# rsjahnige/CRYSTALS-Kyber

Hardware: AMD Instinct MI355X
Metric: ML-KEM-768 encaps+decaps/sec at batch 2^20; achieved HBM GB/s vs peak (higher is better)
Workload: dtype u32+f32 (64-bit Keccak lanes as 2 x u32; mod-3329 arithmetic exact on integers < 2^24 in the fp32 pipe; u8/u16 I/O)

## Files before the change

### crystals-kyber_amd/csrc/mlkem_keyset.hpp

```cpp
#pragma once
#include "mlkem_pipeline.hpp"

namespace mlkem {

constexpr int32_t KS_ERR_ARG = -101;

struct KeysetView {
    const uint8_t* keys = nullptr;
    size_t key_stride = 0;
    size_t ek_off = 0;
    const uint8_t* h = nullptr;
    const uint16_t* At = nullptr;
    size_t n_keys = 0;
    bool has_dk = false;
};

struct KeysetLimits {
    size_t enc_max_k[3] = {1536, 1024, 768}, dec_max_k[3] = {3072, 2048, 3072};
    size_t enc_lat_k[3] = {256, 512, 256}, dec_lat_k[3] = {384, 256, 256};
    size_t enc_max(int k) const { return enc_max_k[k - 2]; }
    size_t dec_max(int k) const { return dec_max_k[k - 2]; }
    size_t enc_lat(int k) const { return enc_lat_k[k - 2]; }
    size_t dec_lat(int k) const { return dec_lat_k[k - 2]; }
    void set_all(size_t max_items, size_t lat_items) {
        for (int i = 0; i < 3; i++) {
            if (max_items != (size_t)-1) enc_max_k[i] = dec_max_k[i] = max_items;
            if (lat_items != (size_t)-1) enc_lat_k[i] = dec_lat_k[i] = lat_items;
        }
    }
};

__device__ __forceinline__ size_t keyset_key(const uint32_t* __restrict__ idx, size_t n_keys, size_t item) {
    if (!idx) return 0;
    const size_t k = idx[item];
    return k < n_keys ? k : 0;
}

__global__ void __launch_bounds__(WAVE, MLKEM_KECCAK_MINWAVES) k_hash_g_keyset(size_t n, const uint32_t* __restrict__ idx, size_t n_keys,
                                                                               const uint8_t* __restrict__ m, const uint8_t* __restrict__ hs,
                                                                               uint8_t* __restrict__ Kout, uint8_t* __restrict__ r_ws) {
    const size_t item = (size_t)blockIdx.x * WAVE + lane_id();
    const size_t it = item < n ? item : n - 1;
    uint32_t mm[8], hh[8], w[8];
    load32(m, 32, it, mm);
    load32(hs, 32, keyset_key(idx, n_keys, it), hh);
    KeccakState s;
    lane_G64(s, mm, hh);
    if (item < n) {
        MLKEM_STATE_WORDS8(s, 0, w)
        store32(Kout, 32, item, w);
        MLKEM_STATE_WORDS8(s, 8, w)
        store32(r_ws, 32, item, w);
    }
}

__global__ void __launch_bounds__(256) k_keyset_gather32(size_t n, const uint32_t* __restrict__ idx, size_t n_keys, const uint8_t* __restrict__ src,
                                                         size_t stride, uint32_t* __restrict__ dst) {
    const size_t g = (size_t)blockIdx.x * blockDim.x + threadIdx.x;
    if (g >= 8 * n) return;
    const size_t item = g >> 3;
    dst[g] = reinterpret_cast<const uint32_t*>(src + keyset_key(idx, n_keys, item) * stride)[g & 7];
}

template <int K, int CLEN, int JRATE>
__global__ void __launch_bounds__(WAVE, MLKEM_KECCAK_MINWAVES) k_hash_decaps_keyset(size_t n, const uint32_t* __restrict__ idx, size_t n_keys,
                                                                                    const uint8_t* __restrict__ hs, uint8_t* __restrict__ z_ws,
                                                                                    const uint8_t* __restrict__ c, const uint8_t* __restrict__ m_ws,
                                                                                    uint8_t* __restrict__ Kp_ws, uint8_t* __restrict__ r_ws,
                                                                                    uint8_t* __restrict__ Kbar_ws) {
    __shared__ __attribute__((aligned(16))) uint2 stage[STAGE_QWORDS];
    const size_t item0 = (size_t)blockIdx.x * WAVE;
    KeccakState s;
    uint32_t h[8], w[8];
    {
        MsgView mv{z_ws, 32, 32, c, CLEN, CLEN};
        wave_sponge_absorb<JRATE, 0x1F>(s, stage, mv, item0, n);
        const size_t i2 = item0 + (size_t)lane_id_fresh();
        if (i2 < n) {
            MLKEM_STATE_WORDS8(s, 0, w)
            store32(Kbar_ws, 32, i2, w);
            uint32_t* zr = reinterpret_cast<uint32_t*>(z_ws + i2 * 32);
#pragma unroll
            for (int q = 0; q < 8; q++) zr[q] = 0u;
        }
    }
    uint32_t mm[8];
    const size_t i3 = item0 + (size_t)lane_id_fresh(), it = i3 < n ? i3 : n - 1;
    load32(m_ws, 32, it, mm);
    load32(hs, 32, keyset_key(idx, n_keys, it), h);
    lane_G64(s, mm, h);
    const size_t item = item0 + (size_t)lane_id_fresh();
    if (item < n) {
        MLKEM_STATE_WORDS8(s, 0, w)
        store32(Kp_ws, 32, item, w);
        MLKEM_STATE_WORDS8(s, 8, w)
        store32(r_ws, 32, item, w);
    }
}

template <int K, int ETA1, int DU, int DV, bool COMPARE>
__global__ void __launch_bounds__(WAVE * KPKE2_WAVES, kpke2_minwaves(K))
k_encrypt2_keyset(size_t n, const uint32_t* __restrict__ idx, size_t n_keys, const uint8_t* __restrict__ ek, size_t ek_stride,
                  const uint16_t* __restrict__ At, const uint8_t* __restrict__ msg, const uint8_t* __restrict__ prf, uint8_t* __restrict__ c_out,
                  const uint8_t* __restrict__ c_in, const uint8_t* __restrict__ Kp, const uint8_t* __restrict__ Kbar, uint8_t* __restrict__ Kout) {
    __shared__ K2Lds<K + 1> lds_all[KPKE2_WAVES];
    const int wv = wave_id();
    const size_t item0 = 2 * ((size_t)blockIdx.x * KPKE2_WAVES + wv);
    if (item0 >= n) return;
    const size_t h = (size_t)(lane_id() >> 5), item = item0 + h < n ? item0 + h : item0;
    const size_t key = keyset_key(idx, n_keys, item);
    encrypt2_body<K, ETA1, DU, DV, COMPARE>(lds_all[wv].xch, item0, n, ek + key * ek_stride, 0, msg, At + key * (size_t)(K * K * 256), prf,
                                            c_out, c_in, Kp, Kbar, Kout, (int32_t*)nullptr, 0);
}

template <int K, int DU, int DV>
__global__ void __launch_bounds__(64 * KPKE4_WAVES, kpke4_minwaves(K)) k_decrypt4_keyset(size_t n, const uint32_t* __restrict__ idx, size_t n_keys,
                                                                                       const uint8_t* __restrict__ dk, size_t dk_stride,
                                                                                       const uint8_t* __restrict__ c, uint8_t* __restrict__ m_out) {
    const size_t quad = (size_t)blockIdx.x * KPKE4_WAVES + wave_id();
    if (4 * quad >= n) return;
    const size_t item_raw = 4 * quad + (size_t)rntt_lane().p, item = item_raw < n ? item_raw : n - 1;
    decrypt4_body<K, DU, DV>(quad, n, dk + keyset_key(idx, n_keys, item) * dk_stride, 0, c, m_out);
}

__global__ void __launch_bounds__(256) k_keyset_fix(size_t n, const uint32_t* __restrict__ idx, size_t n_keys, uint8_t* __restrict__ c,
                                                    unsigned c_len, uint8_t* __restrict__ Kout, int32_t* __restrict__ status) {
    for (size_t i = (size_t)blockIdx.x * blockDim.x + threadIdx.x; i < n; i += (size_t)gridDim.x * blockDim.x) {
        const bool bad = idx && (size_t)idx[i] >= n_keys;
        if (status) status[i] = bad ? KS_ERR_ARG : 0;
        if (!bad) continue;
        uint32_t* k = reinterpret_cast<uint32_t*>(Kout + i * 32);
        for (int w = 0; w < 8; w++) k[w] = 0;
        if (c) {
            uint32_t* cw = reinterpret_cast<uint32_t*>(c + i * c_len);
            for (unsigned w = 0; w < c_len / 4; w++) cw[w] = 0;
        }
    }
}

__global__ void __launch_bounds__(256) k_keyset_status_or(size_t n, const int32_t* __restrict__ status, uint32_t* __restrict__ out) {
    uint32_t v = 0;
    for (size_t i = (size_t)blockIdx.x * blockDim.x + threadIdx.x; i < n; i += (size_t)gridDim.x * blockDim.x) v |= (uint32_t)status[i];
    if (v) atomicOr(out, v);
}

template <int K, int ETA1>
struct __attribute__((aligned(16))) KeysetHand {
    uint8_t prf[(2 * K + 1) * (ETA1 == 3 ? 192 : 128)];
    uint8_t r[32], m[32], Kp[32], Kbar[32];
};

__device__ __forceinline__ void keyset_small_reject(size_t item, uint8_t* c, unsigned c_len, uint8_t* Kout, int32_t* status) {
    const unsigned l = (unsigned)lane_id();
    if (l < 8) reinterpret_cast<uint32_t*>(Kout + item * 32)[l] = 0;
    if (c)
        for (unsigned w = l; w < c_len / 4; w += WAVE) reinterpret_cast<uint32_t*>(c + item * c_len)[w] = 0;
    if (l == 0 && status) status[item] = KS_ERR_ARG;
}

template <int K, int ETA1, int DU, int DV, int NW>
__global__ void __launch_bounds__(WAVE * NW)
k_encaps_keyset_small(size_t n, const uint32_t* __restrict__ idx, size_t n_keys, const uint8_t* __restrict__ ek, size_t ek_stride,
                      const uint8_t* __restrict__ hs, const uint16_t* __restrict__ At, const uint8_t* __restrict__ m, uint8_t* __restrict__ c,
                      uint8_t* __restrict__ Kout, int32_t* __restrict__ status, int prf_rate) {
    __shared__ K2Lds<K + 1> xl;
    __shared__ KeysetHand<K, ETA1> hand;
    __shared__ uint2 rc_tables[NW][WK_RC_ENTRIES];
    __shared__ SmallSync sy;
    constexpr unsigned CLEN = 32 * (DU * K + DV);
    const int wv = wave_id();
    const size_t item = blockIdx.x;
    if (item >= n) return;
    const size_t key = idx ? (size_t)idx[item] : 0;
    if (key >= n_keys) {
        if (wv == 0) keyset_small_reject(item, c, CLEN, Kout, status);
        return;
    }
    const uint8_t* my_ek = ek + key * ek_stride;
    WkLane cst;
    wk_lane_init(cst, rc_tables[wave_id()]);
    if (threadIdx.x == 0) { sy.next_job = K * K; sy.jobs_done = 0; sy.r_ready = 0; sy.kbar_ready = 0; }
    block_barrier();
    if (wv == 0) {
        const int i = wk_index();
        uint2 v;
        v.x = 0; v.y = 0;
        if (i >= 0 && i < 4) v = reinterpret_cast<const uint2*>(m + item * 32)[i];
        else if (i >= 4 && i < 8) v = reinterpret_cast<const uint2*>(hs + key * 32)[i - 4];
        WkState a;
        a.lo = v.x; a.hi = v.y;
        if (i == 8) { a.lo = 0x06u; a.hi = 0x80000000u; }
        wk_permute(a, cst);
        uint2 o;
        o.x = a.lo; o.y = a.hi;
        if (wk_primary() && i < 4) reinterpret_cast<uint2*>(Kout + item * 32)[i] = o;
        else if (wk_primary() && i < 8) reinterpret_cast<uint2*>(hand.r)[i - 4] = o;
        flag_signal(&sy.r_ready);
    }
    small_jobs<K, ETA1>(sy, cst, nullptr, true, nullptr, hand.r, hand.prf, 2 * K + 1, (unsigned)prf_rate, nullptr);
    if (wv != 0) return;
    flag_wait(&sy.jobs_done, (uint32_t)(2 * K + 1));
    encrypt1_body<K, ETA1, DU, DV, false>(xl.xch, my_ek, m + item * 32, At + key * (size_t)(K * K * 256), hand.prf, c + item * CLEN, nullptr,
                                          nullptr, nullptr, nullptr, nullptr);
    if (lane_id() == 0 && status) status[item] = 0;
    wave_lds_fence();
    wave_zero_lds(hand);
    wave_zero_lds(xl);
#ifdef MLKEM_EMU_LDS_PROBE
    if (lane_id() == 0) { MLKEM_EMU_LDS_PROBE(&hand, sizeof hand); MLKEM_EMU_LDS_PROBE(&xl, sizeof xl); }
#endif
}

template <int K, int ETA1, int DU, int DV, int JRATE, int NW>
__global__ void __launch_bounds__(WAVE * NW)
k_decaps_keyset_small(size_t n, const uint32_t* __restrict__ idx, size_t n_keys, const uint8_t* __restrict__ dk, size_t dk_stride,
                      const uint8_t* __restrict__ hs, const uint16_t* __restrict__ At, const uint8_t* __restrict__ c, uint8_t* __restrict__ Kout,
                      int32_t* __restrict__ status, int prf_rate) {
    static_assert(NW >= 2, "roles of waves 0 and 1");
    __shared__ K2Lds<K + 1> xl;
    __shared__ KeysetHand<K, ETA1> hand;
    __shared__ uint2 rc_tables[NW][WK_RC_ENTRIES];
    __shared__ SmallSync sy;
    constexpr unsigned DK = 768 * K + 96, CLEN = 32 * (DU * K + DV);
    const int wv = wave_id();
    const size_t item = blockIdx.x;
    if (item >= n) return;
    const size_t key = idx ? (size_t)idx[item] : 0;
    if (key >= n_keys) {
        if (wv == 0) keyset_small_reject(item, nullptr, CLEN, Kout, status);
        return;
    }
    const uint8_t* my_dk = dk + key * dk_stride;
    const uint8_t* my_c = c + item * CLEN;
    WkLane cst;
    wk_lane_init(cst, rc_tables[wave_id()]);
    const int i = wk_index();
    const bool prim = wk_primary();
    if (threadIdx.x == 0) { sy.next_job = K * K; sy.jobs_done = 0; sy.r_ready = 0; sy.kbar_ready = 0; }
    block_barrier();
    if (wv == 0) {
        decrypt4_body<K, DU, DV>(0, 1, my_dk, (size_t)DK, my_c, hand.m);
        wave_global_fence();
        uint2 v;
        v.x = 0; v.y = 0;
        if (i >= 0 && i < 4) v = reinterpret_cast<const uint2*>(hand.m)[i];
        else if (i >= 4 && i < 8) v = reinterpret_cast<const uint2*>(hs + key * 32)[i - 4];
        WkState a;
        a.lo = v.x; a.hi = v.y;
        if (i == 8) { a.lo = 0x06u; a.hi = 0x80000000u; }
        wk_permute(a, cst);
        uint2 o;
        o.x = a.lo; o.y = a.hi;
        if (prim && i < 4) reinterpret_cast<uint2*>(hand.Kp)[i] = o;
        else if (prim && i < 8) reinterpret_cast<uint2*>(hand.r)[i - 4] = o;
        flag_signal(&sy.r_ready);
    } else if (wv == 1) {
        WkState a;
        wk_absorb<JRATE, 0x1F>(a, cst, my_dk + 768 * K + 64, 32, my_c, 32 + CLEN);
        uint2 o;
        o.x = a.lo; o.y = a.hi;
        if (prim && i < 4) reinterpret_cast<uint2*>(hand.Kbar)[i] = o;
        flag_signal(&sy.kbar_ready);
    }
    small_jobs<K, ETA1>(sy, cst, nullptr, true, nullptr, hand.r, hand.prf, 2 * K + 1, (unsigned)prf_rate, nullptr);
    if (wv != 0) return;
    flag_wait(&sy.jobs_done, (uint32_t)(2 * K + 1));
    encrypt1_body<K, ETA1, DU, DV, true>(xl.xch, my_dk + 384 * K, hand.m, At + key * (size_t)(K * K * 256), hand.prf, nullptr, my_c, hand.Kp,
                                         hand.Kbar, Kout + item * 32, nullptr, &sy.kbar_ready);
    if (lane_id() == 0 && status) status[item] = 0;
    wave_lds_fence();
    wave_zero_lds(hand);
    wave_zero_lds(xl);
#ifdef MLKEM_EMU_LDS_PROBE
    if (lane_id() == 0) { MLKEM_EMU_LDS_PROBE(&hand, sizeof hand); MLKEM_EMU_LDS_PROBE(&xl, sizeof xl); }
#endif
}

inline size_t keyset_table_bytes_per_key(const ParamSet& p, bool has_dk) {
    return (has_dk ? (size_t)p.dk_len : (size_t)p.ek_len) + 32 + (size_t)(p.k * p.k) * 512;
}

template <int K>
inline void keyset_import_run(stream_t st, const ParamSet& p, const KeysetView& ks, uint8_t* hs, uint16_t* At, int32_t* status,
                              uint32_t* status_or, const Workspace& ws) {
    const size_t n = ks.n_keys;
    zero_u32x2(st, status_or);
    if (status) {
        const uint8_t* ek = ks.has_dk ? nullptr : ks.keys;
        const uint8_t* dk = ks.has_dk ? ks.keys : nullptr;
        check_keys_dispatch(st, p.set, n, ek, dk, nullptr, nullptr, status, nullptr, min_sz(n, ws.cap), ws);
        launch("k_keyset_status_or", k_keyset_status_or, min_sz(ceil_div(n, 256), 1024), 256u, st, n, (const int32_t*)status, status_or);
    }
    hash_launch(st, 0, n, ks.keys + ks.ek_off, p.ek_len, ks.key_stride, hs);
    for (size_t c0 = 0; c0 < n; c0 += ws.cap) {
        const size_t cn = min_sz(ws.cap, n - c0);
        Workspace w = ws;
        w.A = At + c0 * (size_t)(K * K * 256);
        launch_sample_split(st, p, cn, 0, ks.keys + c0 * ks.key_stride + ks.ek_off + 384 * K, ks.key_stride, 1, nullptr, 0, 0, w);
    }
}

inline void keyset_seed_run(stream_t st, const ParamSet& p, size_t n, const uint8_t* seed, uint8_t* dk, uint8_t* tmp, const Workspace& ws) {
    uint8_t *d = tmp, *z = d + n * 32, *ek = z + n * 32;
    launch("k_seed_split", k_seed_split, ceil_div(4 * n, 256), 256, st, n, reinterpret_cast<const uint4*>(seed), reinterpret_cast<uint4*>(d),
           reinterpret_cast<uint4*>(z));
    keygen_dispatch(st, p.set, n, d, z, ek, dk, ws);
}

template <int K, int ETA1, int DU, int DV>
inline void encaps_keyset_run(stream_t st, const ParamSet& p, const KeysetView& ks, size_t n, const uint32_t* idx, const uint8_t* m, uint8_t* c,
                              uint8_t* Kout, int32_t* status, const Workspace& ws, const KeysetLimits& lim) {
    if (n == 0) return;
    const uint8_t* ek = ks.keys + ks.ek_off;
    if (n <= lim.enc_max(K)) {
        const int rate = ws.fips ? 136 : 168;
        if (n <= lim.enc_lat(K))
            launch("k_encaps_keyset_small", k_encaps_keyset_small<K, ETA1, DU, DV, SMALL_WAVES>, n, WAVE * SMALL_WAVES, st, n, idx, ks.n_keys, ek,
                   ks.key_stride, ks.h, ks.At, m, c, Kout, status, rate);
        else
            launch("k_encaps_keyset_small", k_encaps_keyset_small<K, ETA1, DU, DV, SMALL_WAVES_DENSE>, n, WAVE * SMALL_WAVES_DENSE, st, n, idx,
                   ks.n_keys, ek, ks.key_stride, ks.h, ks.At, m, c, Kout, status, rate);
        return;
    }
    for (size_t h0 = 0; h0 < n; h0 += ws.hcap) {
        const size_t hn = min_sz(ws.hcap, n - h0);
        const uint32_t* idh = idx ? idx + h0 : nullptr;
        launch("k_hash_g_keyset", k_hash_g_keyset, ceil_div(hn, WAVE), WAVE, st, hn, idh, ks.n_keys, m + h0 * 32, ks.h, Kout + h0 * 32, ws.r);
        for (size_t c0 = 0; c0 < hn; c0 += ws.cap) {
            const size_t cn = min_sz(ws.cap, hn - c0), i0 = h0 + c0;
            launch_sample_split(st, p, 0, cn, nullptr, 0, 1, ws.r + c0 * 32, 2 * K + 1, K, ws);
            launch("k_encrypt_keyset", k_encrypt2_keyset<K, ETA1, DU, DV, false>, ceil_div(ceil_div(cn, 2), KPKE2_WAVES), WAVE * KPKE2_WAVES, st, cn,
                   idx ? idx + i0 : nullptr, ks.n_keys, ek, ks.key_stride, ks.At, m + i0 * 32, (const uint8_t*)ws.prf, c + i0 * p.c_len,
                   (const uint8_t*)nullptr, (const uint8_t*)nullptr, (const uint8_t*)nullptr, (uint8_t*)nullptr);
        }
    }
    if (idx || status)
        launch("k_keyset_fix", k_keyset_fix, min_sz(ceil_div(n, 256), 1024), 256u, st, n, idx, ks.n_keys, c, p.c_len, Kout, status);
}

template <int K, int ETA1, int DU, int DV>
inline void decaps_keyset_run(stream_t st, const ParamSet& p, const KeysetView& ks, size_t n, const uint32_t* idx, const uint8_t* c,
                              uint8_t* Kout, int32_t* status, const Workspace& ws, const KeysetLimits& lim) {
    constexpr int CLEN = 32 * (DU * K + DV);
    if (n == 0) return;
    if (n <= lim.dec_max(K)) {
        const int rate = ws.fips ? 136 : 168;
#define MLKEM_DKS(JR, NW) launch("k_decaps_keyset_small", k_decaps_keyset_small<K, ETA1, DU, DV, JR, NW>, n, WAVE * NW, st, n, idx, ks.n_keys, \
                                 ks.keys, ks.key_stride, ks.h, ks.At, c, Kout, status, rate)
        if (!ws.fips && n <= lim.dec_lat(K)) MLKEM_DKS(168, SMALL_WAVES);
        else if (!ws.fips) MLKEM_DKS(168, SMALL_WAVES_DENSE);
        else if (n <= lim.dec_lat(K)) MLKEM_DKS(136, SMALL_WAVES);
        else MLKEM_DKS(136, SMALL_WAVES_DENSE);
#undef MLKEM_DKS
        return;
    }
    for (size_t h0 = 0; h0 < n; h0 += ws.hcap) {
        const size_t hn = min_sz(ws.hcap, n - h0);
        const uint32_t* idh = idx ? idx + h0 : nullptr;
        const uint8_t* ch = c + h0 * p.c_len;
        launch("k_decrypt_keyset", k_decrypt4_keyset<K, DU, DV>, ceil_div(ceil_div(hn, 4), KPKE4_WAVES), 64 * KPKE4_WAVES, st, hn, idh, ks.n_keys,
               ks.keys, ks.key_stride, ch, ws.m);
        launch("k_keyset_gather32", k_keyset_gather32, ceil_div(8 * hn, 256), 256u, st, hn, idh, ks.n_keys, ks.keys + 768 * K + 64, ks.key_stride,
               reinterpret_cast<uint32_t*>(ws.rho));
        if (!ws.fips)
            launch("k_hash_decaps_keyset", k_hash_decaps_keyset<K, CLEN, 168>, ceil_div(hn, WAVE), WAVE, st, hn, idh, ks.n_keys, ks.h,
                   ws.rho, ch, (const uint8_t*)ws.m, ws.Kp, ws.r, ws.Kbar);
        else
            launch("k_hash_decaps_keyset", k_hash_decaps_keyset<K, CLEN, 136>, ceil_div(hn, WAVE), WAVE, st, hn, idh, ks.n_keys, ks.h,
                   ws.rho, ch, (const uint8_t*)ws.m, ws.Kp, ws.r, ws.Kbar);
        for (size_t c0 = 0; c0 < hn; c0 += ws.cap) {
            const size_t cn = min_sz(ws.cap, hn - c0), i0 = h0 + c0;
            launch_sample_split(st, p, 0, cn, nullptr, 0, 1, ws.r + c0 * 32, 2 * K + 1, K, ws);
            launch("k_encrypt_cmp_keyset", k_encrypt2_keyset<K, ETA1, DU, DV, true>, ceil_div(ceil_div(cn, 2), KPKE2_WAVES), WAVE * KPKE2_WAVES, st,
                   cn, idx ? idx + i0 : nullptr, ks.n_keys, ks.keys + 384 * K, ks.key_stride, ks.At, (const uint8_t*)(ws.m + c0 * 32),
                   (const uint8_t*)ws.prf, (uint8_t*)nullptr, c + i0 * p.c_len, (const uint8_t*)(ws.Kp + c0 * 32), (const uint8_t*)(ws.Kbar + c0 * 32),
                   Kout + i0 * 32);
        }
    }
    if (idx || status)
        launch("k_keyset_fix", k_keyset_fix, min_sz(ceil_div(n, 256), 1024), 256u, st, n, idx, ks.n_keys, (uint8_t*)nullptr, p.c_len, Kout, status);
}

inline int keyset_import_dispatch(stream_t st, const ParamSet& p, const KeysetView& ks, uint8_t* hs, uint16_t* At, int32_t* status,
                                  uint32_t* status_or, const Workspace& ws) {
    switch (p.set) {
    case 512: keyset_import_run<2>(st, p, ks, hs, At, status, status_or, ws); break;
    case 768: keyset_import_run<3>(st, p, ks, hs, At, status, status_or, ws); break;
    default: keyset_import_run<4>(st, p, ks, hs, At, status, status_or, ws); break;
    }
    return 0;
}
inline int encaps_keyset_dispatch(stream_t st, const ParamSet& p, const KeysetView& ks, size_t n, const uint32_t* idx, const uint8_t* m,
                                  uint8_t* c, uint8_t* K, int32_t* status, const Workspace& ws, const KeysetLimits& lim) {
    switch (p.set) {
    case 512: encaps_keyset_run<2, 3, 10, 4>(st, p, ks, n, idx, m, c, K, status, ws, lim); break;
    case 768: encaps_keyset_run<3, 2, 10, 4>(st, p, ks, n, idx, m, c, K, status, ws, lim); break;
    default: encaps_keyset_run<4, 2, 11, 5>(st, p, ks, n, idx, m, c, K, status, ws, lim); break;
    }
    return 0;
}
inline int decaps_keyset_dispatch(stream_t st, const ParamSet& p, const KeysetView& ks, size_t n, const uint32_t* idx, const uint8_t* c,
                                  uint8_t* K, int32_t* status, const Workspace& ws, const KeysetLimits& lim) {
    switch (p.set) {
    case 512: decaps_keyset_run<2, 3, 10, 4>(st, p, ks, n, idx, c, K, status, ws, lim); break;
    case 768: decaps_keyset_run<3, 2, 10, 4>(st, p, ks, n, idx, c, K, status, ws, lim); break;
    default: decaps_keyset_run<4, 2, 11, 5>(st, p, ks, n, idx, c, K, status, ws, lim); break;
    }
    return 0;
}

}
```

### crystals-kyber_amd/csrc/mlkem_kpke2.hpp

```cpp
#pragma once
#include "mlkem_arith.hpp"
#include "mlkem_rntt.hpp"
#include <type_traits>

namespace mlkem {

#ifndef MLKEM_KPKE2_WAVES
#define MLKEM_KPKE2_WAVES 1
#endif
constexpr int KPKE2_WAVES = MLKEM_KPKE2_WAVES;
#ifdef MLKEM_KPKE2_MINWAVES
constexpr int kpke2_minwaves(int) { return MLKEM_KPKE2_MINWAVES; }
#else
constexpr int kpke2_minwaves(int k) { return k == 2 ? 4 : k == 3 ? 3 : 2; }
#endif

template <int NP>
struct __attribute__((aligned(16))) K2Lds {
    float2 xch[NP][2][128];
};

__device__ __forceinline__ int k2_slot(int pair) { return pair ^ ((pair & 64) ? 0x15 : 0) ^ ((pair & 32) ? 0x0A : 0); }
enum K2Layout { K2_LA = 0, K2_LB = 1, K2_LC = 2, K2_NAT = 3 };
__device__ __forceinline__ int k2_blk(int t) { return (((t >> 2) & 3) << 3) | ((t >> 4) << 2) | (t & 3); }
__device__ __forceinline__ int k2_lc_hi(int t) { return (((t >> 2) & 3) << 2) | ((t >> 4) << 1) | ((t >> 1) & 1); }
template <int LAYOUT>
__device__ __forceinline__ int k2_pair(int t, int j) {
    if constexpr (LAYOUT == K2_LA) return (j << 5) | t;
    else if constexpr (LAYOUT == K2_LB) return ((t >> 3) << 5) | (j << 3) | (t & 7);
    else if constexpr (LAYOUT == K2_LC) return (k2_lc_hi(t) << 3) | (j << 1) | (t & 1);
    else return (k2_blk(t) << 2) | j;
}
template <int LAYOUT>
__device__ __forceinline__ void k2_write(float2* xh, int t, const v2f (&p)[4]) {
#pragma unroll
    for (int j = 0; j < 4; j++) {
        float2 v;
        v.x = p[j].x; v.y = p[j].y;
        xh[k2_slot(k2_pair<LAYOUT>(t, j))] = v;
    }
}
template <int LAYOUT>
__device__ __forceinline__ void k2_read(const float2* xh, int t, v2f (&p)[4]) {
#pragma unroll
    for (int j = 0; j < 4; j++) {
        const float2 v = xh[k2_slot(k2_pair<LAYOUT>(t, j))];
        p[j] = v2f{v.x, v.y};
    }
}
template <int FROM, int TO, int NP>
__device__ __forceinline__ void k2_exchange(float2 (*xch)[2][128], int h, int t, v2f (&p)[NP][4]) {
#pragma unroll
    for (int q = 0; q < NP; q++) k2_write<FROM>(xch[q][h], t, p[q]);
    wave_lds_fence();
#pragma unroll
    for (int q = 0; q < NP; q++) k2_read<TO>(xch[q][h], t, p[q]);
    wave_lds_fence();
}

struct K2Tw {
    Tw b0, b1, b2, c0, c1, c2, d0, d1;
};
__device__ __forceinline__ void k2_twiddles_fwd(K2Tw& w, int t) {
    const Tw* z = ZETA_F.z;
    const int b = t >> 3, c = k2_lc_hi(t), n = k2_blk(t);
    w.b0 = z[4 + b]; w.b1 = z[8 + 2 * b]; w.b2 = z[9 + 2 * b];
    w.c0 = z[16 + c]; w.c1 = z[32 + 2 * c]; w.c2 = z[33 + 2 * c];
    w.d0 = z[64 + 2 * n]; w.d1 = z[65 + 2 * n];
}
__device__ __forceinline__ void k2_twiddles_inv(K2Tw& w, int t) {
    const Tw* z = ZETA_F.z;
    const int b = t >> 3, c = k2_lc_hi(t), n = k2_blk(t);
    w.d0 = z[127 - 2 * n]; w.d1 = z[126 - 2 * n];
    w.c1 = z[63 - 2 * c]; w.c2 = z[62 - 2 * c]; w.c0 = z[31 - c];
    w.b1 = z[15 - 2 * b]; w.b2 = z[14 - 2 * b]; w.b0 = z[7 - b];
}

template <int N>
__device__ __forceinline__ void k2_shoup_n(const Tw (&z)[N], v2f (&b)[N]) {
    v2f km[N], nk[N];
#pragma unroll
    for (int i = 0; i < N; i++) km[i] = fma2(b[i], splat2(z[i].zq), splat2(F_MAGIC));
#pragma unroll
    for (int i = 0; i < N; i++) nk[i] = fma2(km[i], splat2(-F_Q), splat2(F_MAGIC_Q));
#pragma unroll
    for (int i = 0; i < N; i++) b[i] = fma2(b[i], splat2(z[i].z), nk[i]);
}
template <int N>
__device__ __forceinline__ void k2_fred_n(v2f (&x)[N]) {
    v2f k[N];
#pragma unroll
    for (int i = 0; i < N; i++) k[i] = fma2(x[i], splat2(F_INVQ), splat2(F_MAGIC));
#pragma unroll
    for (int i = 0; i < N; i++) k[i] = k[i] - splat2(F_MAGIC);
#pragma unroll
    for (int i = 0; i < N; i++) x[i] = fma2(k[i], splat2(-F_Q), x[i]);
}
template <int N, bool GS>
__device__ __forceinline__ void k2_bfly_n(v2f (&a)[N], v2f (&b)[N], const Tw (&z)[N]) {
    if constexpr (!GS) {
        k2_shoup_n<N>(z, b);
#pragma unroll
        for (int i = 0; i < N; i++) { const v2f tt = b[i]; b[i] = a[i] - tt; a[i] = a[i] + tt; }
    } else {
        v2f d[N];
#pragma unroll
        for (int i = 0; i < N; i++) d[i] = b[i] - a[i];
#pragma unroll
        for (int i = 0; i < N; i++) a[i] = a[i] + b[i];
        k2_shoup_n<N>(z, d);
#pragma unroll
        for (int i = 0; i < N; i++) b[i] = d[i];
    }
}
template <int NP, bool GS>
__device__ __forceinline__ void k2_layer_hi(v2f (&p)[NP][4], Tw z) {
    v2f a[2 * NP], b[2 * NP];
    Tw zz[2 * NP];
#pragma unroll
    for (int q = 0; q < NP; q++) { a[2 * q] = p[q][0]; b[2 * q] = p[q][2]; a[2 * q + 1] = p[q][1]; b[2 * q + 1] = p[q][3]; zz[2 * q] = z; zz[2 * q + 1] = z; }
    k2_bfly_n<2 * NP, GS>(a, b, zz);
#pragma unroll
    for (int q = 0; q < NP; q++) { p[q][0] = a[2 * q]; p[q][2] = b[2 * q]; p[q][1] = a[2 * q + 1]; p[q][3] = b[2 * q + 1]; }
}
template <int NP, bool GS>
__device__ __forceinline__ void k2_layer_lo(v2f (&p)[NP][4], Tw z01, Tw z23) {
    v2f a[2 * NP], b[2 * NP];
    Tw zz[2 * NP];
#pragma unroll
    for (int q = 0; q < NP; q++) { a[2 * q] = p[q][0]; b[2 * q] = p[q][1]; a[2 * q + 1] = p[q][2]; b[2 * q + 1] = p[q][3]; zz[2 * q] = z01; zz[2 * q + 1] = z23; }
    k2_bfly_n<2 * NP, GS>(a, b, zz);
#pragma unroll
    for (int q = 0; q < NP; q++) { p[q][0] = a[2 * q]; p[q][1] = b[2 * q]; p[q][2] = a[2 * q + 1]; p[q][3] = b[2 * q + 1]; }
}
template <int NP, int R0, int R1>
__device__ __forceinline__ void k2_fred_pairs(v2f (&p)[NP][4]) {
    v2f x[2 * NP];
#pragma unroll
    for (int q = 0; q < NP; q++) { x[2 * q] = p[q][R0]; x[2 * q + 1] = p[q][R1]; }
    k2_fred_n<2 * NP>(x);
#pragma unroll
    for (int q = 0; q < NP; q++) { p[q][R0] = x[2 * q]; p[q][R1] = x[2 * q + 1]; }
}

template <int NP>
__device__ __forceinline__ void k2_ntt(v2f (&p)[NP][4], float2 (*xch)[2][128], int h, int t, const K2Tw& w) {
    k2_layer_hi<NP, false>(p, FZ1);
    k2_layer_lo<NP, false>(p, FZ2, FZ3);
    k2_exchange<K2_LA, K2_LB, NP>(xch, h, t, p);
    k2_layer_hi<NP, false>(p, w.b0);
    k2_layer_lo<NP, false>(p, w.b1, w.b2);
    k2_exchange<K2_LB, K2_LC, NP>(xch, h, t, p);
    k2_layer_hi<NP, false>(p, w.c0);
    k2_layer_lo<NP, false>(p, w.c1, w.c2);
    k2_exchange<K2_LC, K2_NAT, NP>(xch, h, t, p);
    k2_layer_lo<NP, false>(p, w.d0, w.d1);
}
template <int NP>
__device__ __forceinline__ void k2_intt(v2f (&p)[NP][4], float2 (*xch)[2][128], int h, int t, const K2Tw& w) {
    k2_layer_lo<NP, true>(p, w.d0, w.d1);
    k2_fred_pairs<NP, 0, 2>(p);
    k2_exchange<K2_NAT, K2_LC, NP>(xch, h, t, p);
    k2_layer_lo<NP, true>(p, w.c1, w.c2);
    k2_layer_hi<NP, true>(p, w.c0);
    k2_fred_pairs<NP, 0, 1>(p);
    k2_exchange<K2_LC, K2_LB, NP>(xch, h, t, p);
    k2_layer_lo<NP, true>(p, w.b1, w.b2);
    k2_layer_hi<NP, true>(p, w.b0);
    k2_fred_pairs<NP, 0, 1>(p);
    k2_exchange<K2_LB, K2_LA, NP>(xch, h, t, p);
    k2_layer_lo<NP, true>(p, FZ3, FZ2);
    {
        v2f sm[2 * NP], df[2 * NP];
        Tw zs[2 * NP], zd[2 * NP];
#pragma unroll
        for (int q = 0; q < NP; q++)
#pragma unroll
            for (int m = 0; m < 2; m++) {
                sm[2 * q + m] = p[q][m] + p[q][m + 2];
                df[2 * q + m] = p[q][m + 2] - p[q][m];
                zs[2 * q + m] = F_INV128; zd[2 * q + m] = F_INV128_Z1;
            }
        k2_shoup_n<2 * NP>(zs, sm);
        k2_shoup_n<2 * NP>(zd, df);
#pragma unroll
        for (int q = 0; q < NP; q++)
#pragma unroll
            for (int m = 0; m < 2; m++) { p[q][m] = sm[2 * q + m]; p[q][m + 2] = df[2 * q + m]; }
    }
    k2_exchange<K2_LA, K2_NAT, NP>(xch, h, t, p);
}

template <int ETA>
struct K2CbdRaw {
    uint32_t w[ETA == 2 ? 1 : 2];
};
template <int ETA>
__device__ __forceinline__ void k2_cbd_load_la(const uint8_t* prf, int t, K2CbdRaw<ETA>& r) {
    if constexpr (ETA == 2) {
        r.w[0] = (uint32_t)prf[t] | ((uint32_t)prf[t + 32] << 8) | ((uint32_t)prf[t + 64] << 16) | ((uint32_t)prf[t + 96] << 24);
    } else {
        uint32_t f[4];
#pragma unroll
        for (int j = 0; j < 4; j++) {
            const int o = ((3 * t) >> 1) + 48 * j;
            f[j] = (((uint32_t)prf[o] | ((uint32_t)prf[o + 1] << 8)) >> (4 * (t & 1))) & 0xFFFu;
        }
        r.w[0] = f[0] | (f[1] << 12);
        r.w[1] = f[2] | (f[3] << 12);
    }
}
__device__ __forceinline__ uint32_t k2_cbd_load_nat2(const uint8_t* prf, int t) { return reinterpret_cast<const uint32_t*>(prf)[t]; }
template <bool BIASED = false>
__device__ __forceinline__ void k2_cbd2_eval8(uint32_t t, v2f (&p)[4]) {
    const uint32_t s = (t & 0x55555555u) + ((t >> 1) & 0x55555555u);
    const uint32_t d = ((s & 0x33333333u) + 0x22222222u) - ((s >> 2) & 0x33333333u);
    const uint32_t lo = d & 0x0F0F0F0Fu, hi = (d >> 4) & 0x0F0F0F0Fu;
    float fl[4] = {(float)(lo & 0xFFu), (float)((lo >> 8) & 0xFFu), (float)((lo >> 16) & 0xFFu), (float)(lo >> 24)};
    float fh[4] = {(float)(hi & 0xFFu), (float)((hi >> 8) & 0xFFu), (float)((hi >> 16) & 0xFFu), (float)(hi >> 24)};
#ifndef MLKEM_EMU
    asm volatile("" : "+v"(fl[0]), "+v"(fl[1]), "+v"(fl[2]), "+v"(fl[3]), "+v"(fh[0]), "+v"(fh[1]), "+v"(fh[2]), "+v"(fh[3]));
#endif
#pragma unroll
    for (int j = 0; j < 4; j++) {
        if constexpr (BIASED) p[j] = v2f{fl[j], fh[j]};
        else p[j] = v2f{fl[j], fh[j]} - splat2(2.0f);
    }
}
template <int ETA>
__device__ __forceinline__ void k2_cbd_eval(const K2CbdRaw<ETA>& r, v2f (&p)[4]) {
    if constexpr (ETA == 2) {
        k2_cbd2_eval8<false>(r.w[0], p);
    } else {
        float a[4], b[4];
        cbd_eval_f<3>(r.w[0], a);
        cbd_eval_f<3>(r.w[1], b);
        p[0] = v2f{a[0], a[1]}; p[1] = v2f{a[2], a[3]}; p[2] = v2f{b[0], b[1]}; p[3] = v2f{b[2], b[3]};
    }
}

__device__ __forceinline__ void k2_gamma(const v2f (&y)[4], Tw d0, Tw d1, float (&yg)[4]) {
    yg[0] = fmulmod_shoup(d0, y[0].y);
    yg[1] = fmulmod_shoup(tw_neg(d0), y[1].y);
    yg[2] = fmulmod_shoup(d1, y[2].y);
    yg[3] = fmulmod_shoup(tw_neg(d1), y[3].y);
}
__device__ __forceinline__ void k2_basemul_acc(v2f (&acc)[4], const v2f (&a)[4], const v2f (&y)[4], const float (&yg)[4]) {
    v2f c[4];
#pragma unroll
    for (int j = 0; j < 4; j++) c[j] = fma2(splat2(a[j].x), y[j], acc[j]);
#pragma unroll
    for (int j = 0; j < 4; j++) {
        c[j].x = __builtin_fmaf(a[j].y, yg[j], c[j].x);
        c[j].y = __builtin_fmaf(a[j].y, y[j].x, c[j].y);
    }
    k2_fred_n<4>(c);
#pragma unroll
    for (int j = 0; j < 4; j++) acc[j] = c[j];
}

__device__ __forceinline__ void k2_unpack16(const uint4 v, v2f (&p)[4]) {
    const uint32_t w[4] = {v.x, v.y, v.z, v.w};
#pragma unroll
    for (int j = 0; j < 4; j++) p[j] = v2f{(float)(w[j] & 0xFFFFu), (float)(w[j] >> 16)};
}
__device__ __forceinline__ void k2_decode12(uint32_t w0, uint32_t w1, uint32_t w2, v2f (&p)[4]) {
    const uint32_t c0 = w0 & 0xFFFu, c1 = (w0 >> 12) & 0xFFFu, c2 = __builtin_amdgcn_alignbit(w1, w0, 24) & 0xFFFu, c3 = (w1 >> 4) & 0xFFFu;
    const uint32_t c4 = (w1 >> 16) & 0xFFFu, c5 = __builtin_amdgcn_alignbit(w2, w1, 28) & 0xFFFu, c6 = (w2 >> 8) & 0xFFFu, c7 = w2 >> 20;
    p[0] = v2f{(float)c0, (float)c1}; p[1] = v2f{(float)c2, (float)c3}; p[2] = v2f{(float)c4, (float)c5}; p[3] = v2f{(float)c6, (float)c7};
}

__device__ __forceinline__ uint32_t f_bits(float x) {
    union { float f; uint32_t u; } v;
    v.f = x;
    return v.u;
}
template <int D, bool BIASED = false>
__device__ __forceinline__ void k2_compress4(const v2f (&x)[4], unsigned (&c)[8]) {
    v2f tt[4], k0m[4], k0[4], r[4], km[4];
#pragma unroll
    for (int j = 0; j < 4; j++) tt[j] = fma2(x[j], splat2((float)(1 << D)), splat2(BIASED ? -(float)(2 << D) : 0.0f));
#pragma unroll
    for (int j = 0; j < 4; j++) k0m[j] = fma2(tt[j], splat2(F_INVQ), splat2(F_MAGIC));
#pragma unroll
    for (int j = 0; j < 4; j++) k0[j] = k0m[j] - splat2(F_MAGIC);
#pragma unroll
    for (int j = 0; j < 4; j++) r[j] = fma2(k0[j], splat2(-F_Q), tt[j]);
#pragma unroll
    for (int j = 0; j < 4; j++) km[j] = fma2(r[j], splat2(F_INVQ), splat2(F_MAGIC));
#pragma unroll
    for (int j = 0; j < 4; j++) {
        c[2 * j] = (f_bits(k0m[j].x) + f_bits(km[j].x)) & ((1u << D) - 1u);
        c[2 * j + 1] = (f_bits(k0m[j].y) + f_bits(km[j].y)) & ((1u << D) - 1u);
    }
}

__device__ __forceinline__ uint32_t k2_swap1(uint32_t v) {
#ifdef MLKEM_EMU
    return (uint32_t)emu_quad_shfl((int)v, (int)((threadIdx.x & 3) ^ 1));
#else
    return (uint32_t)__builtin_amdgcn_mov_dpp((int)v, 0xB1, 0xF, 0xF, true);
#endif
}
__device__ __forceinline__ uint32_t k2_prev_in_quad(uint32_t v) {
#ifdef MLKEM_EMU
    const int l = (int)(threadIdx.x & 3);
    return (uint32_t)emu_quad_shfl((int)v, l ? l - 1 : l);
#else
    return (uint32_t)__builtin_amdgcn_mov_dpp((int)v, 0x90, 0xF, 0xF, true);
#endif
}
__device__ __forceinline__ uint32_t k2_shl_hi(uint32_t hi, uint32_t lo, unsigned s) {
    return s ? __builtin_amdgcn_alignbit(hi, lo, 32u - s) : hi;
}

template <int D>
struct K2Piece {
    static_assert(D == 4 || D == 5 || D == 10 || D == 11 || D == 12, "ciphertext / key encodings of ML-KEM");
    static constexpr int NW = D == 4 ? 1 : D == 5 ? 2 : 3;
    uint32_t w[NW];
    static __device__ __forceinline__ int first(int t) {
        if constexpr (D == 4) return t;
        else if constexpr (D == 12) return 3 * t;
        else if constexpr (D == 10) return 5 * (t >> 1) + ((t & 1) ? 3 : 0);
        else if constexpr (D == 11) return 11 * (t >> 2) + ((88 * (t & 3)) >> 5);
        else return 5 * (t >> 2) + (t & 3);
    }
    static __device__ __forceinline__ int count(int t) {
        if constexpr (D == 4) return 1;
        else if constexpr (D == 12) return 3;
        else if constexpr (D == 10) return (t & 1) ? 2 : 3;
        else if constexpr (D == 11) return (t & 3) ? 3 : 2;
        else return (t & 3) == 3 ? 2 : 1;
    }
};
template <int D>
__device__ __forceinline__ void k2_encode(const unsigned (&c)[8], int t, K2Piece<D>& o) {
    if constexpr (D == 4) {
        o.w[0] = c[0] | (c[1] << 4) | (c[2] << 8) | (c[3] << 12) | (c[4] << 16) | (c[5] << 20) | (c[6] << 24) | (c[7] << 28);
    } else if constexpr (D == 12) {
        o.w[0] = c[0] | (c[1] << 12) | (c[2] << 24);
        o.w[1] = (c[2] >> 8) | (c[3] << 4) | (c[4] << 16) | (c[5] << 28);
        o.w[2] = (c[5] >> 4) | (c[6] << 8) | (c[7] << 20);
    } else if constexpr (D == 10) {
        const uint32_t v0 = c[0] | (c[1] << 10) | (c[2] << 20) | (c[3] << 30);
        const uint32_t v1 = (c[3] >> 2) | (c[4] << 8) | (c[5] << 18) | (c[6] << 28);
        const uint32_t v2 = (c[6] >> 4) | (c[7] << 6);
        const uint32_t other0 = k2_swap1(v0);
        const unsigned sh = (t & 1) ? 16u : 0u;
        o.w[0] = __builtin_amdgcn_alignbit(v1, v0, sh);
        o.w[1] = __builtin_amdgcn_alignbit(v2, v1, sh);
        o.w[2] = v2 | (other0 << 16);
    } else if constexpr (D == 11) {
        const uint32_t v0 = c[0] | (c[1] << 11) | (c[2] << 22);
        const uint32_t v1 = (c[2] >> 10) | (c[3] << 1) | (c[4] << 12) | (c[5] << 23);
        const uint32_t v2 = (c[5] >> 9) | (c[6] << 2) | (c[7] << 13);
        const int j = t & 3;
        const unsigned sh = (88u * (unsigned)j) & 31u;
        const uint32_t e0 = v0 << sh, e1 = k2_shl_hi(v1, v0, sh), e2 = k2_shl_hi(v2, v1, sh), e3 = k2_shl_hi(0u, v2, sh);
        const uint32_t tail = j == 0 ? e2 : e3;
        const uint32_t prev = k2_prev_in_quad(tail);
        o.w[0] = e0 | (j ? prev : 0u);
        o.w[1] = e1;
        o.w[2] = e2;
    } else {
        const uint32_t v0 = c[0] | (c[1] << 5) | (c[2] << 10) | (c[3] << 15) | (c[4] << 20) | (c[5] << 25) | (c[6] << 30);
        const uint32_t v1 = (c[6] >> 2) | (c[7] << 3);
        const int j = t & 3;
        const unsigned sh = 8u * (unsigned)j;
        const uint32_t e0 = v0 << sh, e1 = k2_shl_hi(v1, v0, sh);
        const uint32_t prev = k2_prev_in_quad(e1);
        o.w[0] = e0 | (j ? prev : 0u);
        o.w[1] = e1;
    }
}
template <int D>
__device__ __forceinline__ void k2_piece_load(const uint8_t* poly, int t, K2Piece<D>& o) {
    const uint32_t* g = reinterpret_cast<const uint32_t*>(poly) + K2Piece<D>::first(t);
#pragma unroll
    for (int i = 0; i < K2Piece<D>::NW; i++) o.w[i] = i < K2Piece<D>::count(t) ? stream_load4(g + i) : 0u;
}
template <int D>
__device__ __forceinline__ void k2_piece_store(uint8_t* poly, int t, const K2Piece<D>& o) {
    uint32_t* g = reinterpret_cast<uint32_t*>(poly) + K2Piece<D>::first(t);
#pragma unroll
    for (int i = 0; i < K2Piece<D>::NW; i++)
        if (i < K2Piece<D>::count(t)) g[i] = o.w[i];
}
template <int D>
__device__ __forceinline__ uint32_t k2_piece_diff(int t, const K2Piece<D>& a, const K2Piece<D>& ref) {
    uint32_t d = 0;
#pragma unroll
    for (int i = 0; i < K2Piece<D>::NW; i++)
        if (i < K2Piece<D>::count(t)) d |= a.w[i] ^ ref.w[i];
    return d;
}
template <int D, bool COMPARE, bool BIASED = false>
__device__ __forceinline__ uint32_t k2_emit(const v2f (&p)[4], int t, uint8_t* out, const K2Piece<D>& ref, bool store) {
    unsigned c[8];
    k2_compress4<D, BIASED>(p, c);
    K2Piece<D> o;
    k2_encode<D>(c, t, o);
    if constexpr (COMPARE) return k2_piece_diff<D>(t, o, ref);
    if (store) k2_piece_store<D>(out, t, o);
    return 0;
}

template <int K, int ETA1, int DU, int DV, bool COMPARE>
__device__ __forceinline__ void
encrypt2_body(float2 (*xch)[2][128], size_t item0, size_t n, const uint8_t* __restrict__ ek, size_t ek_stride, const uint8_t* __restrict__ msg,
              const uint16_t* __restrict__ A, const uint8_t* __restrict__ prf, uint8_t* __restrict__ c_out, const uint8_t* __restrict__ c_in,
              const uint8_t* __restrict__ Kp, const uint8_t* __restrict__ Kbar, uint8_t* __restrict__ Kout, int32_t* __restrict__ mod_status,
              size_t a_stride) {
    const int l = lane_id(), h = l >> 5, t = l & 31, nb = k2_blk(t);
    const bool valid = item0 + (size_t)h < n;
    const unsigned hh = valid ? (unsigned)h : 0u;
    constexpr unsigned PS = (ETA1 == 3) ? 192 : 128, CLEN = 32 * (DU * K + DV), PRFLEN = (2 * K + 1) * PS;
    const uint8_t* my_prf = prf + item0 * (size_t)PRFLEN + (size_t)(hh * PRFLEN);
    const uint8_t* my_ek = ek + item0 * ek_stride + (size_t)(hh * (unsigned)ek_stride);
    const uint16_t* my_A = A + item0 * a_stride + (size_t)(hh * (unsigned)a_stride);
    uint8_t* my_c = COMPARE ? nullptr : c_out + item0 * CLEN + (size_t)(hh * CLEN);
    const uint8_t* my_cin = COMPARE ? c_in + item0 * CLEN + (size_t)(hh * CLEN) : nullptr;
    const size_t item = item0 + hh;

    K2CbdRaw<ETA1> raw_y[K];
#pragma unroll
    for (int b = 0; b < K; b++) k2_cbd_load_la<ETA1>(my_prf + b * PS, t, raw_y[b]);
    uint4 a_all[K + 1][K];
#pragma unroll
    for (int a = 0; a < K; a++)
#pragma unroll
        for (int b = 0; b < K; b++) a_all[a][b] = *reinterpret_cast<const uint4*>(my_A + (a * K + b) * 256 + 8 * nb);
#pragma unroll
    for (int b = 0; b < K; b++) {
        const uint32_t* gp = reinterpret_cast<const uint32_t*>(my_ek + 384 * b) + 3 * nb;
        a_all[K][b].x = stream_load4(gp); a_all[K][b].y = stream_load4(gp + 1); a_all[K][b].z = stream_load4(gp + 2); a_all[K][b].w = 0u;
    }
    uint32_t raw_e[K + 1];
#pragma unroll
    for (int a = 0; a <= K; a++) raw_e[a] = k2_cbd_load_nat2(my_prf + (K + a) * PS, nb);
    const unsigned mb = msg[item * 32 + nb];

    v2f yh[K][4];
    float yg[K][4];
    {
        K2Tw tw;
        k2_twiddles_fwd(tw, t);
#pragma unroll
        for (int b = 0; b < K; b++) k2_cbd_eval<ETA1>(raw_y[b], yh[b]);
        k2_ntt<K>(yh, xch, h, t, tw);
#pragma unroll
        for (int b = 0; b < K; b++) {
            k2_fred_n<4>(yh[b]);
            k2_gamma(yh[b], tw.d0, tw.d1, yg[b]);
        }
    }
    uint32_t diff = 0;
    bool over = false;
    constexpr int NG = K + 1;
    v2f acc[NG][4];
    K2Piece<DU> cu_ref[NG];
    K2Piece<DV> cv_ref;
#pragma unroll
    for (int a = 0; a < NG; a++) {
#pragma unroll
        for (int j = 0; j < 4; j++) acc[a][j] = splat2(0.f);
#pragma unroll
        for (int b = 0; b < K; b++) {
            v2f av[4];
            if (a < K) {
                k2_unpack16(a_all[a][b], av);
            } else {
                k2_decode12(a_all[a][b].x, a_all[a][b].y, a_all[a][b].z, av);
#pragma unroll
                for (int j = 0; j < 4; j++) over = over || (av[j].x >= F_Q) || (av[j].y >= F_Q);
            }
            k2_basemul_acc(acc[a], av, yh[b], yg[b]);
        }
    }
    if constexpr (COMPARE) {
#pragma unroll
        for (int a = 0; a < NG; a++) {
            if (a < K) k2_piece_load<DU>(my_cin + a * 32 * DU, nb, cu_ref[a]);
            else k2_piece_load<DV>(my_cin + K * 32 * DU, nb, cv_ref);
        }
    }
    {
        K2Tw twi;
        k2_twiddles_inv(twi, t);
        k2_intt<NG>(acc, xch, h, t, twi);
    }
#pragma unroll
    for (int a = 0; a < NG; a++) {
        v2f e[4];
        k2_cbd2_eval8<true>(raw_e[a], e);
#pragma unroll
        for (int j = 0; j < 4; j++) acc[a][j] = acc[a][j] + e[j];
        if (a < K) {
            diff |= k2_emit<DU, COMPARE, true>(acc[a], nb, COMPARE ? nullptr : my_c + a * 32 * DU, cu_ref[a], valid);
        } else {
#pragma unroll
            for (int j = 0; j < 4; j++)
                acc[a][j] = acc[a][j] + v2f{((mb >> (2 * j)) & 1u) ? 1665.0f : 0.0f, ((mb >> (2 * j + 1)) & 1u) ? 1665.0f : 0.0f};
            diff |= k2_emit<DV, COMPARE, true>(acc[a], nb, COMPARE ? nullptr : my_c + K * 32 * DU, cv_ref, valid);
        }
    }
    if (mod_status) {
        const unsigned long long bal = __ballot(over);
        const bool bad = ((bal >> (32 * h)) & 0xFFFFFFFFull) != 0;
        if (t == 0 && valid) mod_status[item] = bad ? -4 : 0;
    }
    if constexpr (COMPARE) {
        const unsigned long long bal = __ballot(diff != 0);
        const uint32_t reject = ((bal >> (32 * h)) & 0xFFFFFFFFull) != 0 ? 0xFFFFFFFFu : 0u;
        if (t < 8 && valid) {
            const uint32_t kp = reinterpret_cast<const uint32_t*>(Kp + item * 32)[t];
            const uint32_t kb = reinterpret_cast<const uint32_t*>(Kbar + item * 32)[t];
            reinterpret_cast<uint32_t*>(Kout + item * 32)[t] = (kp & ~reject) | (kb & reject);
        }
    }
}
template <int K, int ETA1, int DU, int DV, bool COMPARE, bool A_T = false>
__device__ __forceinline__ void
encrypt1_body(float2 (*xch)[2][128], const uint8_t* __restrict__ ek, const uint8_t* __restrict__ msg, const uint16_t* __restrict__ A,
              const uint8_t* __restrict__ prf, uint8_t* __restrict__ c_out, const uint8_t* __restrict__ c_in, const uint8_t* __restrict__ Kp,
              const uint8_t* Kbar, uint8_t* __restrict__ Kout, int32_t* __restrict__ mod_status,
              const uint32_t* kbar_flag = nullptr) {
    const int l = lane_id(), h = l >> 5, t = l & 31, nb = k2_blk(t);
    constexpr unsigned PS = (ETA1 == 3) ? 192 : 128;
    constexpr int NG = K + 1, NL = (NG + 1) / 2;
    auto kind = [](int i) constexpr { return 2 * i + 1 < K ? 0 : (2 * i < K ? 1 : 2); };

    K2CbdRaw<ETA1> raw_y[K];
#pragma unroll
    for (int b = 0; b < K; b++) k2_cbd_load_la<ETA1>(prf + b * PS, t, raw_y[b]);
    uint4 a_all[NL][K];
    uint32_t raw_e[NL];
#pragma unroll
    for (int i = 0; i < NL; i++) {
        const int a = kind(i) == 2 ? K : 2 * i + h;
        const bool is_v = kind(i) == 2 || (kind(i) == 1 && h == 1);
#pragma unroll
        for (int b = 0; b < K; b++) {
            if (is_v) {
                const uint32_t* gp = reinterpret_cast<const uint32_t*>(ek + 384 * b) + 3 * nb;
                a_all[i][b].x = gp[0]; a_all[i][b].y = gp[1]; a_all[i][b].z = gp[2]; a_all[i][b].w = 0u;
            } else {
                a_all[i][b] = *reinterpret_cast<const uint4*>(A + (A_T ? b * K + a : a * K + b) * 256 + 8 * nb);
            }
        }
        raw_e[i] = k2_cbd_load_nat2(prf + (K + a) * PS, nb);
    }
    const unsigned mb = msg[nb];

    v2f yh[K][4];
    float yg[K][4];
    {
        K2Tw tw;
        k2_twiddles_fwd(tw, t);
#pragma unroll
        for (int b = 0; b < K; b++) k2_cbd_eval<ETA1>(raw_y[b], yh[b]);
        k2_ntt<K>(yh, xch, h, t, tw);
#pragma unroll
        for (int b = 0; b < K; b++) {
            k2_fred_n<4>(yh[b]);
            k2_gamma(yh[b], tw.d0, tw.d1, yg[b]);
        }
    }
    uint32_t diff = 0;
    bool over = false;
    v2f acc[NL][4];
    K2Piece<DU> cu_ref[NL];
    K2Piece<DV> cv_ref;
#pragma unroll
    for (int i = 0; i < NL; i++) {
        const bool is_v = kind(i) == 2 || (kind(i) == 1 && h == 1);
#pragma unroll
        for (int j = 0; j < 4; j++) acc[i][j] = splat2(0.f);
#pragma unroll
        for (int b = 0; b < K; b++) {
            v2f av[4];
            if (is_v) {
                k2_decode12(a_all[i][b].x, a_all[i][b].y, a_all[i][b].z, av);
#pragma unroll
                for (int j = 0; j < 4; j++) over = over || (av[j].x >= F_Q) || (av[j].y >= F_Q);
            } else {
                k2_unpack16(a_all[i][b], av);
            }
            k2_basemul_acc(acc[i], av, yh[b], yg[b]);
        }
    }
    if constexpr (COMPARE) {
#pragma unroll
        for (int i = 0; i < NL; i++) {
            const int a = kind(i) == 2 ? K : 2 * i + h;
            const bool is_v = kind(i) == 2 || (kind(i) == 1 && h == 1);
            if (is_v) k2_piece_load<DV>(c_in + K * 32 * DU, nb, cv_ref);
            else k2_piece_load<DU>(c_in + a * 32 * DU, nb, cu_ref[i]);
        }
    }
    {
        K2Tw twi;
        k2_twiddles_inv(twi, t);
        k2_intt<NL>(acc, xch, h, t, twi);
    }
#pragma unroll
    for (int i = 0; i < NL; i++) {
        const int a = kind(i) == 2 ? K : 2 * i + h;
        const bool is_v = kind(i) == 2 || (kind(i) == 1 && h == 1);
        const bool store = kind(i) != 2 || h == 0;
        v2f e[4];
        k2_cbd2_eval8<true>(raw_e[i], e);
#pragma unroll
        for (int j = 0; j < 4; j++) acc[i][j] = acc[i][j] + e[j];
        if (is_v) {
#pragma unroll
            for (int j = 0; j < 4; j++)
                acc[i][j] = acc[i][j] + v2f{((mb >> (2 * j)) & 1u) ? 1665.0f : 0.0f, ((mb >> (2 * j + 1)) & 1u) ? 1665.0f : 0.0f};
            diff |= k2_emit<DV, COMPARE, true>(acc[i], nb, COMPARE ? nullptr : c_out + K * 32 * DU, cv_ref, store);
        } else {
            diff |= k2_emit<DU, COMPARE, true>(acc[i], nb, COMPARE ? nullptr : c_out + a * 32 * DU, cu_ref[i], store);
        }
    }
    if (mod_status) {
        const bool bad = __ballot(over) != 0;
        if (l == 0) mod_status[0] = bad ? -4 : 0;
    }
    if constexpr (COMPARE) {
        const uint32_t reject = __ballot(diff != 0) != 0 ? 0xFFFFFFFFu : 0u;
        if (kbar_flag) flag_wait(kbar_flag, 1u);
        if (l < 8) {
            const uint32_t kp = reinterpret_cast<const uint32_t*>(Kp)[l];
            const uint32_t kb = reinterpret_cast<const uint32_t*>(Kbar)[l];
            reinterpret_cast<uint32_t*>(Kout)[l] = (kp & ~reject) | (kb & reject);
        }
    }
}

template <int K, int ETA1, int DU, int DV, bool COMPARE>
__global__ void __launch_bounds__(WAVE * KPKE2_WAVES, kpke2_minwaves(K))
k_encrypt2(size_t n, const uint8_t* __restrict__ ek, size_t ek_stride, const uint8_t* __restrict__ msg, const uint16_t* __restrict__ A,
           const uint8_t* __restrict__ prf, uint8_t* __restrict__ c_out, const uint8_t* __restrict__ c_in, const uint8_t* __restrict__ Kp,
           const uint8_t* __restrict__ Kbar, uint8_t* __restrict__ Kout, int32_t* __restrict__ mod_status, size_t a_stride) {
    __shared__ K2Lds<K + 1> lds_all[KPKE2_WAVES];
    const int wv = wave_id();
    const size_t item0 = 2 * ((size_t)blockIdx.x * KPKE2_WAVES + wv);
    if (item0 >= n) return;
    encrypt2_body<K, ETA1, DU, DV, COMPARE>(lds_all[wv].xch, item0, n, ek, ek_stride, msg, A, prf, c_out, c_in, Kp, Kbar, Kout, mod_status, a_stride);
}

__device__ __forceinline__ void k2_canon(const v2f (&p)[4], unsigned (&c)[8]) {
    v2f r[4] = {p[0], p[1], p[2], p[3]};
    k2_fred_n<4>(r);
#pragma unroll
    for (int j = 0; j < 4; j++) {
        const int a = (int)r[j].x, b = (int)r[j].y;
        c[2 * j] = (unsigned)(a + ((a >> 31) & KQ));
        c[2 * j + 1] = (unsigned)(b + ((b >> 31) & KQ));
    }
}

template <int K, int ETA1, bool KEM_DK>
__device__ __forceinline__ void
keygen2_body(float2 (*xch)[2][128], size_t item0, size_t n, const uint16_t* __restrict__ A, const uint8_t* __restrict__ prf,
             const uint8_t* __restrict__ rho, uint8_t* __restrict__ ek, uint8_t* __restrict__ dk) {
    const int l = lane_id(), h = l >> 5, t = l & 31, nb = k2_blk(t);
    const bool valid = item0 + (size_t)h < n;
    const unsigned hh = valid ? (unsigned)h : 0u;
    constexpr unsigned PS = (ETA1 == 3) ? 192 : 128, EK = 384 * K + 32, DK = KEM_DK ? 768 * K + 96 : 384 * K, PRFLEN = 2 * K * PS;
    const uint8_t* my_prf = prf + item0 * (size_t)PRFLEN + (size_t)(hh * PRFLEN);
    const uint16_t* my_A = A + item0 * (size_t)(K * K * 256) + (size_t)(hh * (unsigned)(K * K * 256));
    uint8_t* my_ek = ek + item0 * EK + (size_t)(hh * EK);
    uint8_t* my_dk = dk + item0 * DK + (size_t)(hh * DK);
    const size_t item = item0 + hh;

    K2CbdRaw<ETA1> raw_s[K], raw_e[K];
#pragma unroll
    for (int b = 0; b < K; b++) k2_cbd_load_la<ETA1>(my_prf + b * PS, t, raw_s[b]);
    constexpr bool PF = K >= 3;
    uint4 a_all[K][K];
    if constexpr (PF) {
#pragma unroll
        for (int a = 0; a < K; a++)
#pragma unroll
            for (int b = 0; b < K; b++) a_all[a][b] = *reinterpret_cast<const uint4*>(my_A + (a * K + b) * 256 + 8 * nb);
    }
#pragma unroll
    for (int a = 0; a < K; a++) k2_cbd_load_la<ETA1>(my_prf + (K + a) * PS, t, raw_e[a]);
    const uint32_t rho_w = reinterpret_cast<const uint32_t*>(rho + item * 32)[t & 7];
    K2Tw tw;
    k2_twiddles_fwd(tw, t);
    v2f sh[K][4];
    float sg[K][4];
#pragma unroll
    for (int b = 0; b < K; b++) k2_cbd_eval<ETA1>(raw_s[b], sh[b]);
    k2_ntt<K>(sh, xch, h, t, tw);
#pragma unroll
    for (int b = 0; b < K; b++) {
        k2_fred_n<4>(sh[b]);
        k2_gamma(sh[b], tw.d0, tw.d1, sg[b]);
        unsigned c[8];
        k2_canon(sh[b], c);
        K2Piece<12> o;
        k2_encode<12>(c, nb, o);
        if (valid) k2_piece_store<12>(my_dk + 384 * b, nb, o);
    }
    v2f eh[K][4];
#pragma unroll
    for (int a = 0; a < K; a++) k2_cbd_eval<ETA1>(raw_e[a], eh[a]);
    k2_ntt<K>(eh, xch, h, t, tw);
#pragma unroll
    for (int a = 0; a < K; a++) {
        v2f acc[4] = {splat2(0.f), splat2(0.f), splat2(0.f), splat2(0.f)};
#pragma unroll
        for (int b = 0; b < K; b++) {
            v2f av[4];
            if constexpr (!PF) a_all[a][b] = *reinterpret_cast<const uint4*>(my_A + (a * K + b) * 256 + 8 * nb);
            k2_unpack16(a_all[a][b], av);
            k2_basemul_acc(acc, av, sh[b], sg[b]);
        }
#pragma unroll
        for (int j = 0; j < 4; j++) acc[j] = acc[j] + eh[a][j];
        unsigned c[8];
        k2_canon(acc, c);
        K2Piece<12> o;
        k2_encode<12>(c, nb, o);
        if (valid) {
            k2_piece_store<12>(my_ek + 384 * a, nb, o);
            if constexpr (KEM_DK) k2_piece_store<12>(my_dk + 384 * K + 384 * a, nb, o);
        }
    }
    if (t < 8 && valid) {
        reinterpret_cast<uint32_t*>(my_ek + 384 * K)[t] = rho_w;
        if constexpr (KEM_DK) reinterpret_cast<uint32_t*>(my_dk + 768 * K)[t] = rho_w;
    }
}
template <int K, int ETA1, bool KEM_DK>
__global__ void __launch_bounds__(WAVE * KPKE2_WAVES, K == 2 ? kpke2_minwaves(2) : kpke2_minwaves(K + 1))
k_keygen2(size_t n, const uint16_t* __restrict__ A, const uint8_t* __restrict__ prf, const uint8_t* __restrict__ rho,
          uint8_t* __restrict__ ek, uint8_t* __restrict__ dk) {
    __shared__ K2Lds<K> lds_all[KPKE2_WAVES];
    const int wv = wave_id();
    const size_t item0 = 2 * ((size_t)blockIdx.x * KPKE2_WAVES + wv);
    if (item0 >= n) return;
    keygen2_body<K, ETA1, KEM_DK>(lds_all[wv].xch, item0, n, A, prf, rho, ek, dk);
}

}
```

### crystals-kyber_amd/csrc/mlkem_pipeline.hpp

```cpp
#pragma once
#include "mlkem_kernels.hpp"
#include "mlkem_sampler.hpp"
#include "mlkem_arith.hpp"
#include "mlkem_rntt.hpp"
#include "mlkem_kpke4.hpp"
#include "mlkem_kpke2.hpp"
#include "mlkem_wkeccak.hpp"
#include "mlkem_small.hpp"
#include "mlkem_check.hpp"
#include <stdlib.h>
#ifndef MLKEM_EMU
#include <vector>
#endif

namespace mlkem {

#ifdef MLKEM_EMU
using stream_t = void*;
#else
using stream_t = hipStream_t;
#endif

#ifndef MLKEM_EMU
struct LaunchRecorder {
    struct Rec { const char* label; hipEvent_t a, b; };
    std::vector<Rec> recs;
    bool failed = false;
};
inline LaunchRecorder*& launch_recorder() {
    static thread_local LaunchRecorder* r = nullptr;
    return r;
}
#endif

template <class... KArgs, class... Args>
inline void launch(const char* label, void (*kfn)(KArgs...), size_t grid, unsigned block, stream_t st, Args... args) {
    if (grid == 0) return;
#ifdef MLKEM_EMU
    (void)st; (void)label;
    emu::launch((unsigned)grid, block, [=] { kfn(args...); });
#else
    LaunchRecorder* rec = launch_recorder();
    LaunchRecorder::Rec r{label, nullptr, nullptr};
    bool timed = rec && hipEventCreate(&r.a) == hipSuccess && hipEventCreate(&r.b) == hipSuccess && hipEventRecord(r.a, st) == hipSuccess;
    kfn<<<dim3((unsigned)grid), dim3(block), 0, st>>>(args...);
    if (timed) timed = hipEventRecord(r.b, st) == hipSuccess;
    if (timed) {
        rec->recs.push_back(r);
    } else if (rec) {
        rec->failed = true;
        if (r.a) (void)hipEventDestroy(r.a);
        if (r.b) (void)hipEventDestroy(r.b);
    }
#endif
}

inline void zero_u32x2(stream_t st, uint32_t* p) {
#ifdef MLKEM_EMU
    (void)st;
    p[0] = 0; p[1] = 0;
#else
    (void)hipMemsetAsync(p, 0, 2 * sizeof(uint32_t), st);
#endif
}

struct ParamSet {
    int set, k, eta1, eta2, du, dv;
    unsigned ek_len, dk_len, c_len;
};
inline bool param_set(int set, ParamSet& p) {
    switch (set) {
    case 512: p = {512, 2, 3, 2, 10, 4, 0, 0, 0}; break;
    case 768: p = {768, 3, 2, 2, 10, 4, 0, 0, 0}; break;
    case 1024: p = {1024, 4, 2, 2, 11, 5, 0, 0, 0}; break;
    default: return false;
    }
    p.ek_len = 384u * p.k + 32;
    p.dk_len = 768u * p.k + 96;
    p.c_len = 32u * (p.du * p.k + p.dv);
    return true;
}

struct Workspace {
    uint16_t* A = nullptr;
    uint8_t *prf = nullptr, *r = nullptr, *rho = nullptr, *m = nullptr, *Kp = nullptr, *Kbar = nullptr;
    uint32_t* leftover = nullptr;
    uint32_t* resume = nullptr;
    uint32_t resume_cap = 0;
    size_t cap = 0;
    size_t hcap = 0;
    size_t wide_max = 2048;
    size_t wide_max_k[3] = {4096, 3072, 4096};
    size_t wide_kem(int k) const { return wide_max_k[k - 2]; }
    size_t small_max_k[3] = {1536, 768, 512};
    size_t small_max(int k) const { return small_max_k[k - 2]; }
    size_t small_lat_max = 256;
    size_t small_wide_max = 128;
    unsigned stages = 15;
    int fips = 0;
#ifndef MLKEM_EMU
    hipStream_t side = nullptr;
    hipEvent_t ev_fork = nullptr, ev_join = nullptr;
    bool side_on = true;
#endif
};
struct SideFork {
    stream_t main, side = nullptr;
#ifndef MLKEM_EMU
    hipEvent_t join = nullptr;
#endif
    SideFork(const Workspace& ws, stream_t st, size_t n) : main(st) {
#ifndef MLKEM_EMU
        if (ws.side && ws.side_on && n <= ws.cap && hipEventRecord(ws.ev_fork, st) == hipSuccess && hipStreamWaitEvent(ws.side, ws.ev_fork, 0) == hipSuccess) {
            side = ws.side;
            join = ws.ev_join;
        }
#else
        (void)ws; (void)n;
#endif
    }
    bool active() const { return side != nullptr; }
    stream_t xof_stream() const { return side ? side : main; }
    void join_main() {
#ifndef MLKEM_EMU
        if (side) {
            if (hipEventRecord(join, side) != hipSuccess || hipStreamWaitEvent(main, join, 0) != hipSuccess) (void)hipStreamSynchronize(side);
            side = nullptr;
        }
#endif
    }
};

inline size_t ceil_div(size_t a, size_t b) { return (a + b - 1) / b; }
inline size_t min_sz(size_t a, size_t b) { return a < b ? a : b; }

template <int QB = KQ, int CAP = SAMPLE_CAP>
inline void launch_sample_split(stream_t st, const ParamSet& p, size_t n_xof_items, size_t n_prf_items, const uint8_t* rho, size_t rho_stride,
                                int transpose, const uint8_t* r, int prf_per_item, int n_eta1, const Workspace& ws) {
    SampleArgs a{};
    a.n_xof = n_xof_items * (size_t)(p.k * p.k);
    a.rho = rho; a.rho_stride = rho_stride; a.K = p.k; a.transpose = transpose; a.A = ws.A;
    a.xof_blocks = (unsigned)ceil_div(a.n_xof, WAVE);
    a.n_prf = n_prf_items * (size_t)prf_per_item;
    a.r = r; a.per_item = prf_per_item; a.n_eta1 = n_eta1; a.eta1 = p.eta1; a.prf = ws.prf;
    a.prf_stride = p.eta1 == 3 ? 192 : 128;
    a.leftover = ws.leftover;
    a.resume = ws.resume;
    a.resume_cap = ws.resume ? ws.resume_cap : 0;
    a.list_mode = 0;
    a.prf_rate = ws.fips ? 136 : 168;
    const size_t grid = a.xof_blocks + ceil_div(a.n_prf, WAVE);
    if (grid == 0) return;
    if (n_xof_items <= ws.wide_kem(p.k) && n_prf_items <= ws.wide_kem(p.k)) {
        launch("k_sample_direct", k_sample<QB, CAP>, grid, WAVE, st, a);
        return;
    }
    if (a.n_xof) zero_u32x2(st, ws.leftover);
    launch("k_sample_main", k_sample_main<QB>, grid, WAVE, st, a);
    if (a.n_xof == 0) return;
    SampleArgs t = a;
    t.list_mode = 1;
    t.n_prf = 0;
    t.xof_blocks = (unsigned)(ceil_div(a.n_xof, WAVE * 16) + 1);
    if (a.resume_cap) {
        launch("k_sample_tail", k_sample_resume<QB, CAP>, (size_t)t.xof_blocks, WAVE, st, t);
        t.xof_blocks = (unsigned)(ceil_div(a.n_xof, WAVE * 256) + 1);
    }
    launch("k_sample_restart", k_sample<QB, CAP>, (size_t)t.xof_blocks, WAVE, st, t);
}
template <int QB = KQ, int CAP = SAMPLE_CAP>
inline void launch_sample(stream_t st, const ParamSet& p, size_t n, const uint8_t* rho, size_t rho_stride, int transpose,
                          const uint8_t* r, int prf_per_item, int n_eta1, const Workspace& ws) {
    launch_sample_split<QB, CAP>(st, p, n, n, rho, rho_stride, transpose, r, prf_per_item, n_eta1, ws);
}

template <int K, int ETA1, int DU, int DV, bool CMP, class... Args>
inline void encrypt_launch(const char* label, stream_t st, size_t n, Args... args) {
    launch(label, k_encrypt2<K, ETA1, DU, DV, CMP>, ceil_div(ceil_div(n, 2), KPKE2_WAVES), WAVE * KPKE2_WAVES, st, n, args...);
}

template <int K, int ETA1>
inline void keygen_run(stream_t st, const ParamSet& p, size_t n, const uint8_t* d, const uint8_t* z, uint8_t* ek, uint8_t* dk,
                       const Workspace& ws) {
    const bool kem = z != nullptr;
    const size_t dk_len = kem ? (size_t)p.dk_len : (size_t)(384 * K);
    if (n && n <= ws.small_max(K)) {
        const int rate = ws.fips ? 136 : 168;
#define MLKEM_KS(KEM, NW) launch("k_keygen_small", k_keygen_small<K, ETA1, KEM, NW>, n, WAVE * NW, st, n, d, z, ek, dk, rate)
        const bool lat = n <= ws.small_lat_max;
        if (kem && lat) MLKEM_KS(true, SMALL_WAVES);
        else if (kem) MLKEM_KS(true, SMALL_WAVES_DENSE);
        else if (lat) MLKEM_KS(false, SMALL_WAVES);
        else MLKEM_KS(false, SMALL_WAVES_DENSE);
#undef MLKEM_KS
        return;
    }
    for (size_t h0 = 0; h0 < n; h0 += ws.hcap) {
        const size_t hn = min_sz(ws.hcap, n - h0);
        launch("k_hash_keygen_seed", k_hash_keygen_seed<K>, ceil_div(hn, WAVE), WAVE, st, hn, d + h0 * 32, ws.rho, ws.r);
        for (size_t c0 = 0; c0 < hn; c0 += ws.cap) {
            const size_t cn = min_sz(ws.cap, hn - c0), i0 = h0 + c0;
            launch_sample(st, p, cn, ws.rho + c0 * 32, 32, 0, ws.r + c0 * 32, 2 * K, 2 * K, ws);
            const size_t kgrid = ceil_div(ceil_div(cn, 2), KPKE2_WAVES);
            if (kem)
                launch("k_keygen", k_keygen2<K, ETA1, true>, kgrid, WAVE * KPKE2_WAVES, st, cn, (const uint16_t*)ws.A, (const uint8_t*)ws.prf,
                       (const uint8_t*)(ws.rho + c0 * 32), ek + i0 * p.ek_len, dk + i0 * dk_len);
            else
                launch("k_keygen", k_keygen2<K, ETA1, false>, kgrid, WAVE * KPKE2_WAVES, st, cn, (const uint16_t*)ws.A, (const uint8_t*)ws.prf,
                       (const uint8_t*)(ws.rho + c0 * 32), ek + i0 * p.ek_len, dk + i0 * dk_len);
        }
        if (kem && n <= ws.wide_kem(K))
            launch("k_hash_keygen_fin", k_hash_keygen_fin_w<K>, hn, WAVE, st, hn, (const uint8_t*)(ek + h0 * p.ek_len), z + h0 * 32, dk + h0 * p.dk_len);
        else if (kem)
            launch("k_hash_keygen_fin", k_hash_keygen_fin<K>, ceil_div(hn, WAVE), WAVE, st, hn, (const uint8_t*)(ek + h0 * p.ek_len),
                   z + h0 * 32, dk + h0 * p.dk_len);
    }
}

template <int K, int ETA1, int DU, int DV>
inline void encaps_run(stream_t st, const ParamSet& p, size_t n, const uint8_t* ek, const uint8_t* m, uint8_t* c, uint8_t* Kout,
                       int32_t* mod_status, const Workspace& ws, const uint8_t* r_user = nullptr) {
    if (n == 0) return;
    if (!r_user && n <= ws.small_max(K)) {
        const int rate = ws.fips ? 136 : 168;
        if (n <= ws.small_lat_max)
            launch("k_encaps_small", k_encaps_small<K, ETA1, DU, DV, SMALL_WAVES>, n, WAVE * SMALL_WAVES, st, n, ek, m, c, Kout, mod_status, rate);
        else
            launch("k_encaps_small", k_encaps_small<K, ETA1, DU, DV, SMALL_WAVES_DENSE>, n, WAVE * SMALL_WAVES_DENSE, st, n, ek, m, c, Kout, mod_status, rate);
        return;
    }
    SideFork fork(ws, st, r_user ? (size_t)-1 : n);
    if (fork.active()) launch_sample_split(fork.xof_stream(), p, n, 0, ek + 384 * K, p.ek_len, 1, nullptr, 2 * K + 1, K, ws);
    for (size_t h0 = 0; h0 < n; h0 += ws.hcap) {
        const size_t hn = min_sz(ws.hcap, n - h0);
        const uint8_t* r_h = r_user ? r_user + h0 * 32 : (const uint8_t*)ws.r;
        if (!(ws.stages & 1u)) {
        } else if (!r_user && n <= ws.wide_kem(K))
            launch("k_hash_encaps", k_hash_encaps_w<K>, hn, WAVE, st, hn, ek + h0 * p.ek_len, m + h0 * 32, Kout + h0 * 32, ws.r);
        else if (!r_user)
            launch("k_hash_encaps", k_hash_encaps<K>, ceil_div(hn, WAVE), WAVE, st, hn, ek + h0 * p.ek_len, m + h0 * 32, Kout + h0 * 32, ws.r);
        for (size_t c0 = 0; c0 < hn; c0 += ws.cap) {
            const size_t cn = min_sz(ws.cap, hn - c0), i0 = h0 + c0;
            const uint8_t* eki = ek + i0 * p.ek_len;
            if (fork.active()) {
                launch_sample_split(st, p, 0, cn, nullptr, 0, 1, r_h + c0 * 32, 2 * K + 1, K, ws);
                fork.join_main();
            } else if (ws.stages & 2u) {
                launch_sample(st, p, cn, eki + 384 * K, p.ek_len, 1, r_h + c0 * 32, 2 * K + 1, K, ws);
            }
            if (ws.stages & 4u)
            encrypt_launch<K, ETA1, DU, DV, false>("k_encrypt", st, cn, eki, (size_t)p.ek_len, m + i0 * 32, (const uint16_t*)ws.A, (const uint8_t*)ws.prf,
                   c + i0 * p.c_len, (const uint8_t*)nullptr, (const uint8_t*)nullptr, (const uint8_t*)nullptr, (uint8_t*)nullptr,
                   mod_status ? mod_status + i0 : (int32_t*)nullptr, (size_t)(K * K * 256));
        }
    }
}

template <int K, int DU, int DV>
inline void decrypt_launch(stream_t st, size_t n, const uint8_t* dk, size_t dk_stride, const uint8_t* c, uint8_t* m) {
    launch("k_decrypt", k_decrypt4<K, DU, DV>, ceil_div(ceil_div(n, 4), KPKE4_WAVES), 64 * KPKE4_WAVES, st, n, dk, dk_stride, c, m);
}

template <int K, int ETA1, int DU, int DV>
inline void decaps_run(stream_t st, const ParamSet& p, size_t n, const uint8_t* dk, const uint8_t* c, uint8_t* Kout,
                       int32_t* status, bool hash_check, const Workspace& ws) {
    constexpr int CLEN = 32 * (DU * K + DV);
    if (n && n <= ws.small_max(K)) {
        const int rate = ws.fips ? 136 : 168;
        int32_t* sts = hash_check ? status : (int32_t*)nullptr;
#define MLKEM_DS(HC, JR, NW) launch("k_decaps_small", k_decaps_small<K, ETA1, DU, DV, HC, JR, NW>, (HC) ? 2 * n : n, WAVE * NW, st, n, dk, c, Kout, sts, rate)
        constexpr int LW = K >= 3 ? SMALL_WAVES_WIDE : SMALL_WAVES;
#define MLKEM_DS2(HC, JR) do { if (n <= ws.small_wide_max) MLKEM_DS(HC, JR, LW); else if (n <= ws.small_lat_max) MLKEM_DS(HC, JR, SMALL_WAVES); else MLKEM_DS(HC, JR, SMALL_WAVES_DENSE); } while (0)
        if (hash_check && !ws.fips) MLKEM_DS2(true, 168);
        else if (!ws.fips) MLKEM_DS2(false, 168);
        else if (hash_check) MLKEM_DS2(true, 136);
        else MLKEM_DS2(false, 136);
#undef MLKEM_DS2
#undef MLKEM_DS
        return;
    }
    for (size_t h0 = 0; h0 < n; h0 += ws.hcap) {
        const size_t hn = min_sz(ws.hcap, n - h0);
        const uint8_t* dkh = dk + h0 * p.dk_len;
        const uint8_t* ch = c + h0 * p.c_len;
        SideFork fork(ws, st, n);
        if (fork.active()) launch_sample_split(fork.xof_stream(), p, n, 0, dk + 768 * K, p.dk_len, 1, nullptr, 2 * K + 1, K, ws);
        if (ws.stages & 8u) decrypt_launch<K, DU, DV>(st, hn, dkh, (size_t)p.dk_len, ch, ws.m);
        int32_t* sth = (hash_check && status) ? status + h0 : (int32_t*)nullptr;
        const size_t hgrid = ceil_div(hn, WAVE);
        if (!(ws.stages & 1u)) {
        } else if (n <= ws.wide_kem(K)) {
            if (hash_check && !ws.fips)
                launch("k_hash_decaps", k_hash_decaps_w<K, CLEN, true, 168>, 2 * hn, WAVE, st, hn, dkh, ch, (const uint8_t*)ws.m, ws.Kp, ws.r, ws.Kbar, sth, (size_t)p.dk_len);
            else if (!ws.fips)
                launch("k_hash_decaps", k_hash_decaps_w<K, CLEN, false, 168>, hn, WAVE, st, hn, dkh, ch, (const uint8_t*)ws.m, ws.Kp, ws.r, ws.Kbar, sth, (size_t)p.dk_len);
            else if (hash_check)
                launch("k_hash_decaps", k_hash_decaps_w<K, CLEN, true, 136>, 2 * hn, WAVE, st, hn, dkh, ch, (const uint8_t*)ws.m, ws.Kp, ws.r, ws.Kbar, sth, (size_t)p.dk_len);
            else
                launch("k_hash_decaps", k_hash_decaps_w<K, CLEN, false, 136>, hn, WAVE, st, hn, dkh, ch, (const uint8_t*)ws.m, ws.Kp, ws.r, ws.Kbar, sth, (size_t)p.dk_len);
        } else
        if (hash_check && !ws.fips)
            launch("k_hash_decaps", k_hash_decaps<K, CLEN, true, 168>, 2 * hgrid, WAVE, st, hn, dkh, ch, (const uint8_t*)ws.m, ws.Kp, ws.r, ws.Kbar, sth, (size_t)p.dk_len);
        else if (!ws.fips)
            launch("k_hash_decaps", k_hash_decaps<K, CLEN, false, 168>, hgrid, WAVE, st, hn, dkh, ch, (const uint8_t*)ws.m, ws.Kp, ws.r, ws.Kbar, sth, (size_t)p.dk_len);
        else if (hash_check)
            launch("k_hash_decaps", k_hash_decaps<K, CLEN, true, 136>, 2 * hgrid, WAVE, st, hn, dkh, ch, (const uint8_t*)ws.m, ws.Kp, ws.r, ws.Kbar, sth, (size_t)p.dk_len);
        else
            launch("k_hash_decaps", k_hash_decaps<K, CLEN, false, 136>, hgrid, WAVE, st, hn, dkh, ch, (const uint8_t*)ws.m, ws.Kp, ws.r, ws.Kbar, sth, (size_t)p.dk_len);
        for (size_t c0 = 0; c0 < hn; c0 += ws.cap) {
            const size_t cn = min_sz(ws.cap, hn - c0), i0 = h0 + c0;
            const uint8_t* dki = dk + i0 * p.dk_len;
            if (fork.active()) {
                launch_sample_split(st, p, 0, cn, nullptr, 0, 1, ws.r + c0 * 32, 2 * K + 1, K, ws);
                fork.join_main();
            } else if (ws.stages & 2u) {
                launch_sample(st, p, cn, dki + 768 * K, p.dk_len, 1, ws.r + c0 * 32, 2 * K + 1, K, ws);
            }
            if (ws.stages & 4u)
            encrypt_launch<K, ETA1, DU, DV, true>("k_encrypt_cmp", st, cn, dki + 384 * K, (size_t)p.dk_len, (const uint8_t*)(ws.m + c0 * 32), (const uint16_t*)ws.A,
                   (const uint8_t*)ws.prf, (uint8_t*)nullptr, c + i0 * p.c_len, (const uint8_t*)(ws.Kp + c0 * 32),
                   (const uint8_t*)(ws.Kbar + c0 * 32), Kout + i0 * 32, (int32_t*)nullptr, (size_t)(K * K * 256));
        }
    }
}

inline size_t seed_stage_bytes(const ParamSet& p) { return 64 + (size_t)p.ek_len + (size_t)p.dk_len; }
template <int K, int ETA1, int DU, int DV>
inline void decaps_seed_run(stream_t st, const ParamSet& p, size_t n, const uint8_t* seed, const uint8_t* c, uint8_t* Kout, uint8_t* stage,
                            size_t stage_items, const Workspace& ws) {
    if (n == 0) return;
    if (n <= ws.small_max(K)) {
        const int rate = ws.fips ? 136 : 168;
#define MLKEM_DSS(JR, NW) launch("k_decaps_seed_small", k_decaps_seed_small<K, ETA1, DU, DV, JR, NW>, n, WAVE * NW, st, n, seed, c, Kout, rate)
#define MLKEM_DSS2(JR) do { if (n <= ws.small_lat_max) MLKEM_DSS(JR, SMALL_WAVES); else MLKEM_DSS(JR, SMALL_WAVES_DENSE); } while (0)
        if (!ws.fips) MLKEM_DSS2(168);
        else MLKEM_DSS2(136);
#undef MLKEM_DSS2
#undef MLKEM_DSS
        return;
    }
    for (size_t s0 = 0; s0 < n; s0 += stage_items) {
        const size_t sn = min_sz(stage_items, n - s0);
        uint8_t *d = stage, *z = d + stage_items * 32, *ek = z + stage_items * 32, *dk = ek + stage_items * p.ek_len;
        launch("k_seed_split", k_seed_split, ceil_div(4 * sn, 256), 256, st, sn, reinterpret_cast<const uint4*>(seed + s0 * 64),
               reinterpret_cast<uint4*>(d), reinterpret_cast<uint4*>(z));
        keygen_run<K, ETA1>(st, p, sn, d, z, ek, dk, ws);
        decaps_run<K, ETA1, DU, DV>(st, p, sn, dk, c + s0 * p.c_len, Kout + s0 * 32, nullptr, false, ws);
    }
}

inline size_t check_stage_bytes(const ParamSet& p, bool has_ek, bool seed, bool pct) {
    return (seed ? seed_stage_bytes(p) : 0) + (pct ? (size_t)p.c_len + 64 + (has_ek ? 0 : (size_t)p.ek_len) : 0);
}
inline size_t check_chunk_items(const ParamSet& p, size_t n, bool has_ek, bool seed, bool pct, size_t stage_bytes, const Workspace& ws) {
    const size_t need = check_stage_bytes(p, has_ek, seed, pct);
    size_t c = min_sz(n, ws.cap);
    if (need) c = min_sz(c, stage_bytes / need);
    return c ? c : 1;
}
template <int K, int ETA1, int DU, int DV>
inline void check_keys_run(stream_t st, const ParamSet& p, size_t n, const uint8_t* ek, const uint8_t* dk, const uint8_t* seed,
                           const uint8_t* m, int32_t* status, uint8_t* stage, size_t chunk, const Workspace& ws) {
    if (n == 0) return;
    const bool hash_in = n <= ws.wide_kem(K);
    for (size_t s0 = 0; s0 < n; s0 += chunk) {
        const size_t sn = min_sz(chunk, n - s0);
        const uint8_t* eki = ek ? ek + s0 * p.ek_len : nullptr;
        const uint8_t* dki = dk ? dk + s0 * p.dk_len : nullptr;
        const uint8_t *sek = nullptr, *sdk = nullptr, *Kc = nullptr, *Kd = nullptr;
        uint8_t* q = stage;
        if (seed) {
            uint8_t *d = q, *z = d + chunk * 32, *e2 = z + chunk * 32, *d2 = e2 + chunk * p.ek_len;
            q = d2 + chunk * p.dk_len;
            launch("k_seed_split", k_seed_split, ceil_div(4 * sn, 256), 256, st, sn, reinterpret_cast<const uint4*>(seed + s0 * 64),
                   reinterpret_cast<uint4*>(d), reinterpret_cast<uint4*>(z));
            keygen_run<K, ETA1>(st, p, sn, d, z, e2, d2, ws);
            sek = e2;
            sdk = d2;
        }
        if (m) {
            const uint8_t* pek = eki;
            if (!ek) {
                uint8_t* g = q;
                q += chunk * p.ek_len;
                launch("k_gather_rows", k_gather_rows, ceil_div(sn * (p.ek_len / 16), 256), 256, st, sn, dki + 384 * K, (size_t)p.dk_len, g,
                       (unsigned)p.ek_len);
                pek = g;
            }
            uint8_t *c = q, *kc = c + chunk * p.c_len, *kd = kc + chunk * 32;
            encaps_run<K, ETA1, DU, DV>(st, p, sn, pek, m + s0 * 32, c, kc, nullptr, ws);
            decaps_run<K, ETA1, DU, DV>(st, p, sn, dki, c, kd, nullptr, false, ws);
            Kc = kc;
            Kd = kd;
        }
        if (hash_in) {
            launch("k_check_keys", k_check_keys<K, true>, sn, 2 * WAVE, st, sn, eki, dki, (const uint8_t*)nullptr, sek, sdk, Kc, Kd, status + s0);
        } else {
            if (dki) launch("k_hash_batch", k_hash_batch<0>, ceil_div(sn, WAVE), WAVE, st, sn, dki + 384 * K, (unsigned)p.ek_len, (size_t)p.dk_len, ws.Kp);
            launch("k_check_keys", k_check_keys<K, false>, ceil_div(sn, 4), WAVE * 4, st, sn, eki, dki, (const uint8_t*)ws.Kp, sek, sdk, Kc, Kd,
                   status + s0);
        }
    }
}

template <int K, int ETA1, int DU, int DV>
inline void encaps_shared_run(stream_t st, const ParamSet& p, size_t n, const uint8_t* ek, const uint8_t* m, uint8_t* c, uint8_t* Kout,
                              const Workspace& ws) {
    const Workspace& w = ws;
    uint8_t* h = ws.rho;
    launch("k_hash_batch", k_hash_batch<0>, (size_t)1, WAVE, st, (size_t)1, ek, (unsigned)p.ek_len, (size_t)p.ek_len, h);
    launch_sample_split(st, p, 1, 0, ek + 384 * K, p.ek_len, 1, nullptr, 0, 0, w);
    for (size_t h0 = 0; h0 < n; h0 += ws.hcap) {
        const size_t hn = min_sz(ws.hcap, n - h0);
        launch("k_hash_g_shared", k_hash_g_shared, ceil_div(hn, WAVE), WAVE, st, hn, m + h0 * 32, (const uint8_t*)h, Kout + h0 * 32, ws.r);
        for (size_t c0 = 0; c0 < hn; c0 += ws.cap) {
            const size_t cn = min_sz(ws.cap, hn - c0), i0 = h0 + c0;
            launch_sample_split(st, p, 0, cn, nullptr, 0, 1, ws.r + c0 * 32, 2 * K + 1, K, w);
            encrypt_launch<K, ETA1, DU, DV, false>("k_encrypt", st, cn, ek, (size_t)0,
                   m + i0 * 32, (const uint16_t*)w.A, (const uint8_t*)w.prf, c + i0 * p.c_len, (const uint8_t*)nullptr,
                   (const uint8_t*)nullptr, (const uint8_t*)nullptr, (uint8_t*)nullptr, (int32_t*)nullptr, (size_t)0);
        }
    }
}
template <int K, int ETA1, int DU, int DV>
inline void decaps_shared_run(stream_t st, const ParamSet& p, size_t n, const uint8_t* dk, const uint8_t* c, uint8_t* Kout,
                              int32_t* status, const Workspace& ws) {
    constexpr int CLEN = 32 * (DU * K + DV);
    const Workspace& w = ws;
    if (status) {
        launch("k_hash_batch", k_hash_batch<0>, (size_t)1, WAVE, st, (size_t)1, dk + 384 * K, (unsigned)p.ek_len, (size_t)p.dk_len, ws.rho);
        launch("k_status_fill", k_status_fill, min_sz(ceil_div(n, 256), 1024), 256u, st, n, (const uint8_t*)ws.rho, dk + 768 * K + 32, status);
    }
    launch_sample_split(st, p, 1, 0, dk + 768 * K, p.dk_len, 1, nullptr, 0, 0, w);
    for (size_t h0 = 0; h0 < n; h0 += ws.hcap) {
        const size_t hn = min_sz(ws.hcap, n - h0);
        const uint8_t* ch = c + h0 * p.c_len;
        decrypt_launch<K, DU, DV>(st, hn, dk, (size_t)0, ch, ws.m);
        const size_t hgrid = ceil_div(hn, WAVE);
        if (!ws.fips)
            launch("k_hash_decaps", k_hash_decaps<K, CLEN, false, 168>, hgrid, WAVE, st, hn, dk, ch, (const uint8_t*)ws.m, ws.Kp, ws.r, ws.Kbar, (int32_t*)nullptr, (size_t)0);
        else
            launch("k_hash_decaps", k_hash_decaps<K, CLEN, false, 136>, hgrid, WAVE, st, hn, dk, ch, (const uint8_t*)ws.m, ws.Kp, ws.r, ws.Kbar, (int32_t*)nullptr, (size_t)0);
        for (size_t c0 = 0; c0 < hn; c0 += ws.cap) {
            const size_t cn = min_sz(ws.cap, hn - c0), i0 = h0 + c0;
            launch_sample_split(st, p, 0, cn, nullptr, 0, 1, ws.r + c0 * 32, 2 * K + 1, K, w);
            encrypt_launch<K, ETA1, DU, DV, true>("k_encrypt_cmp", st, cn, dk + 384 * K,
                   (size_t)0, (const uint8_t*)(ws.m + c0 * 32), (const uint16_t*)w.A, (const uint8_t*)w.prf, (uint8_t*)nullptr, c + i0 * p.c_len,
                   (const uint8_t*)(ws.Kp + c0 * 32), (const uint8_t*)(ws.Kbar + c0 * 32), Kout + i0 * 32, (int32_t*)nullptr, (size_t)0);
        }
    }
}
inline int encaps_shared_dispatch(stream_t st, int set, size_t n, const uint8_t* ek, const uint8_t* m, uint8_t* c, uint8_t* K, const Workspace& ws) {
    ParamSet p;
    if (!param_set(set, p)) return -1;
    if (n == 0) return 0;
    switch (set) {
    case 512: encaps_shared_run<2, 3, 10, 4>(st, p, n, ek, m, c, K, ws); break;
    case 768: encaps_shared_run<3, 2, 10, 4>(st, p, n, ek, m, c, K, ws); break;
    default: encaps_shared_run<4, 2, 11, 5>(st, p, n, ek, m, c, K, ws); break;
    }
    return 0;
}
inline int decaps_shared_dispatch(stream_t st, int set, size_t n, const uint8_t* dk, const uint8_t* c, uint8_t* K, int32_t* status,
                                  const Workspace& ws) {
    ParamSet p;
    if (!param_set(set, p)) return -1;
    if (n == 0) return 0;
    switch (set) {
    case 512: decaps_shared_run<2, 3, 10, 4>(st, p, n, dk, c, K, status, ws); break;
    case 768: decaps_shared_run<3, 2, 10, 4>(st, p, n, dk, c, K, status, ws); break;
    default: decaps_shared_run<4, 2, 11, 5>(st, p, n, dk, c, K, status, ws); break;
    }
    return 0;
}

inline int keygen_dispatch(stream_t st, int set, size_t n, const uint8_t* d, const uint8_t* z, uint8_t* ek, uint8_t* dk,
                           const Workspace& ws) {
    ParamSet p;
    if (!param_set(set, p)) return -1;
    switch (set) {
    case 512: keygen_run<2, 3>(st, p, n, d, z, ek, dk, ws); break;
    case 768: keygen_run<3, 2>(st, p, n, d, z, ek, dk, ws); break;
    default: keygen_run<4, 2>(st, p, n, d, z, ek, dk, ws); break;
    }
    return 0;
}
inline int encaps_dispatch(stream_t st, int set, size_t n, const uint8_t* ek, const uint8_t* m, uint8_t* c, uint8_t* K,
                           int32_t* mod_status, const Workspace& ws) {
    ParamSet p;
    if (!param_set(set, p)) return -1;
    switch (set) {
    case 512: encaps_run<2, 3, 10, 4>(st, p, n, ek, m, c, K, mod_status, ws); break;
    case 768: encaps_run<3, 2, 10, 4>(st, p, n, ek, m, c, K, mod_status, ws); break;
    default: encaps_run<4, 2, 11, 5>(st, p, n, ek, m, c, K, mod_status, ws); break;
    }
    return 0;
}
inline int pke_keygen_dispatch(stream_t st, int set, size_t n, const uint8_t* d, uint8_t* ek, uint8_t* dk_pke, const Workspace& ws) {
    return keygen_dispatch(st, set, n, d, nullptr, ek, dk_pke, ws);
}
inline int pke_encrypt_dispatch(stream_t st, int set, size_t n, const uint8_t* ek, const uint8_t* m, const uint8_t* r, uint8_t* c,
                                const Workspace& ws) {
    ParamSet p;
    if (!param_set(set, p) || !r) return -1;
    switch (set) {
    case 512: encaps_run<2, 3, 10, 4>(st, p, n, ek, m, c, nullptr, nullptr, ws, r); break;
    case 768: encaps_run<3, 2, 10, 4>(st, p, n, ek, m, c, nullptr, nullptr, ws, r); break;
    default: encaps_run<4, 2, 11, 5>(st, p, n, ek, m, c, nullptr, nullptr, ws, r); break;
    }
    return 0;
}
inline int pke_decrypt_dispatch(stream_t st, int set, size_t n, const uint8_t* dk_pke, const uint8_t* c, uint8_t* m) {
    ParamSet p;
    if (!param_set(set, p)) return -1;
    if (n == 0) return 0;
    switch (set) {
    case 512: decrypt_launch<2, 10, 4>(st, n, dk_pke, (size_t)(384 * 2), c, m); break;
    case 768: decrypt_launch<3, 10, 4>(st, n, dk_pke, (size_t)(384 * 3), c, m); break;
    default: decrypt_launch<4, 11, 5>(st, n, dk_pke, (size_t)(384 * 4), c, m); break;
    }
    return 0;
}
inline int decaps_dispatch(stream_t st, int set, size_t n, const uint8_t* dk, const uint8_t* c, uint8_t* K, int32_t* status,
                           bool hash_check, const Workspace& ws) {
    ParamSet p;
    if (!param_set(set, p)) return -1;
    switch (set) {
    case 512: decaps_run<2, 3, 10, 4>(st, p, n, dk, c, K, status, hash_check, ws); break;
    case 768: decaps_run<3, 2, 10, 4>(st, p, n, dk, c, K, status, hash_check, ws); break;
    default: decaps_run<4, 2, 11, 5>(st, p, n, dk, c, K, status, hash_check, ws); break;
    }
    return 0;
}

inline int decaps_seed_dispatch(stream_t st, int set, size_t n, const uint8_t* seed, const uint8_t* c, uint8_t* K, uint8_t* stage,
                                size_t stage_items, const Workspace& ws) {
    ParamSet p;
    if (!param_set(set, p)) return -1;
    switch (set) {
    case 512: decaps_seed_run<2, 3, 10, 4>(st, p, n, seed, c, K, stage, stage_items, ws); break;
    case 768: decaps_seed_run<3, 2, 10, 4>(st, p, n, seed, c, K, stage, stage_items, ws); break;
    default: decaps_seed_run<4, 2, 11, 5>(st, p, n, seed, c, K, stage, stage_items, ws); break;
    }
    return 0;
}

inline int check_keys_dispatch(stream_t st, int set, size_t n, const uint8_t* ek, const uint8_t* dk, const uint8_t* seed, const uint8_t* m,
                               int32_t* status, uint8_t* stage, size_t chunk, const Workspace& ws) {
    ParamSet p;
    if (!param_set(set, p)) return -1;
    switch (set) {
    case 512: check_keys_run<2, 3, 10, 4>(st, p, n, ek, dk, seed, m, status, stage, chunk, ws); break;
    case 768: check_keys_run<3, 2, 10, 4>(st, p, n, ek, dk, seed, m, status, stage, chunk, ws); break;
    default: check_keys_run<4, 2, 11, 5>(st, p, n, ek, dk, seed, m, status, stage, chunk, ws); break;
    }
    return 0;
}

inline size_t poly_grid(size_t n) {
    size_t g = ceil_div(n, ARITH_WAVES);
    const size_t cap = 256 * 16;
    return g < cap ? g : cap;
}
inline size_t ntt_grid_cap() {
    static const size_t v = [] {
        const char* e = getenv("MLKEM_NTT_GRID");
        const long long x = e ? atoll(e) : 0;
        return x > 0 ? (size_t)x : (size_t)(256 * 48);
    }();
    return v;
}
inline void ntt_launch(stream_t st, bool inverse, size_t n, const uint16_t* in, uint16_t* out) {
    size_t grid = ceil_div(ceil_div(n, 4), RNTT_WAVES);
    const size_t cap = ntt_grid_cap();
    if (grid > cap) grid = cap;
    if (inverse) launch("k_intt_batch", k_ntt4_batch<true>, grid, WAVE * RNTT_WAVES, st, n, in, out);
    else launch("k_ntt_batch", k_ntt4_batch<false>, grid, WAVE * RNTT_WAVES, st, n, in, out);
}
inline void basemul_launch(stream_t st, size_t n, const uint16_t* a, const uint16_t* b, uint16_t* h) {
    launch("k_basemul_batch", k_basemul_batch, poly_grid(n), WAVE * ARITH_WAVES, st, n, a, b, h);
}
inline int vecmul_launch(stream_t st, int k, size_t n, const uint16_t* u, const uint16_t* v, uint16_t* w) {
    if (k < 1 || k > 4) return -1;
    launch("k_vecmul_batch", k_vecmul_batch, poly_grid(n), WAVE * ARITH_WAVES, st, n, k, u, v, w);
    return 0;
}
inline void poly_addsub_launch(stream_t st, bool sub, size_t n_values, const uint16_t* a, const uint16_t* b, uint16_t* out) {
    size_t grid = ceil_div(ceil_div(n_values, 8), 256);
    if (grid > 256 * 8) grid = 256 * 8;
    if (sub) launch("k_poly_sub", k_poly_addsub<true>, grid, 256u, st, n_values, a, b, out);
    else launch("k_poly_add", k_poly_addsub<false>, grid, 256u, st, n_values, a, b, out);
}
inline int cbd_launch(stream_t st, int eta, size_t n, const uint8_t* bytes, uint16_t* out) {
    if (eta == 2) launch("k_cbd_batch", k_cbd_batch<2>, poly_grid(n), WAVE * ARITH_WAVES, st, n, bytes, out);
    else if (eta == 3) launch("k_cbd_batch", k_cbd_batch<3>, poly_grid(n), WAVE * ARITH_WAVES, st, n, bytes, out);
    else return -1;
    return 0;
}
inline int codec_launch(stream_t st, bool encode, int d, size_t n, const void* in, void* out) {
#define MLKEM_CODEC_CASE(D)                                                                                                    \
    case D:                                                                                                                    \
        if (encode) launch("k_encode_batch", k_encode_batch<D>, poly_grid(n), WAVE * ARITH_WAVES, st, n, (const uint16_t*)in, (uint8_t*)out); \
        else launch("k_decode_batch", k_decode_batch<D>, poly_grid(n), WAVE * ARITH_WAVES, st, n, (const uint8_t*)in, (uint16_t*)out);        \
        return 0;
    switch (d) {
        MLKEM_CODEC_CASE(1) MLKEM_CODEC_CASE(4) MLKEM_CODEC_CASE(5) MLKEM_CODEC_CASE(10) MLKEM_CODEC_CASE(11) MLKEM_CODEC_CASE(12)
    default: return -1;
    }
#undef MLKEM_CODEC_CASE
}
inline int compress_values_launch(stream_t st, bool decompress, int d, size_t n, const uint16_t* in, uint16_t* out) {
    if (d < 1 || d > 12) return -1;
    size_t grid = ceil_div(ceil_div(n, 8), 256);
    if (grid > 256 * 8) grid = 256 * 8;
    if (grid == 0) return 0;
    if (decompress) launch("k_decompress_values", k_compress_values<true>, grid, 256u, st, n, d, in, out);
    else launch("k_compress_values", k_compress_values<false>, grid, 256u, st, n, d, in, out);
    return 0;
}
template <int QB = KQ, int CAP = SAMPLE_CAP>
inline void sample_ntt_launch(stream_t st, size_t n, const uint8_t* seeds34, uint16_t* out, size_t wave_max = 0, uint8_t* retries = nullptr) {
    if (n <= wave_max) {
        launch("k_sample_xof", k_sample_ntt_w<QB, CAP>, n, WAVE, st, n, seeds34, out, retries);
        return;
    }
    SampleArgs a{};
    a.n_xof = n; a.rho = seeds34; a.rho_stride = 34; a.K = 0; a.A = out; a.retries = retries;
    a.xof_blocks = (unsigned)ceil_div(n, WAVE);
    launch("k_sample_xof", k_sample<QB, CAP>, (size_t)a.xof_blocks, WAVE, st, a);
}
inline int prf_launch(stream_t st, int eta, size_t n, const uint8_t* in33, uint8_t* out) {
    if (eta != 2 && eta != 3) return -1;
    SampleArgs a{};
    a.n_prf = n; a.r = in33; a.per_item = 0; a.eta1 = eta; a.prf = out; a.prf_stride = 64u * (unsigned)eta;
    launch("k_sample_prf", k_sample<>, ceil_div(n, WAVE), WAVE, st, a);
    return 0;
}
inline int hash_launch(stream_t st, int kind, size_t n, const uint8_t* msg, unsigned len, size_t stride, uint8_t* out) {
    if (kind < 0 || kind > 2 || (stride & 7) || stride < len) return -1;
    const size_t grid = ceil_div(n, WAVE);
    if (kind == 0) launch("k_hash_batch", k_hash_batch<0>, grid, WAVE, st, n, msg, len, stride, out);
    else if (kind == 1) launch("k_hash_batch", k_hash_batch<1>, grid, WAVE, st, n, msg, len, stride, out);
    else launch("k_hash_batch", k_hash_batch<2>, grid, WAVE, st, n, msg, len, stride, out);
    return 0;
}

inline void cells_launch(stream_t st, bool to_bytes, size_t n, const void* in, void* out) {
    size_t grid = ceil_div(ceil_div(n, 16), 256);
    if (grid > 256 * 8) grid = 256 * 8;
    if (grid == 0) grid = 1;
    if (to_bytes) launch("k_cells_to_bytes", k_cells_to_bytes, grid, 256u, st, n, (const uint32_t*)in, (uint8_t*)out);
    else launch("k_bytes_to_cells", k_bytes_to_cells, grid, 256u, st, n, (const uint8_t*)in, (uint32_t*)out);
}

inline int sponge_raw_launch(stream_t st, unsigned rate, size_t n, const uint8_t* msg, unsigned nblocks, uint8_t* out, unsigned outlen,
                             size_t out_stride, size_t wave_max = 0) {
    if (nblocks == 0 || out_stride < outlen || rate == 0 || rate >= 200) return -1;
    const bool standard = rate == 72 || rate == 104 || rate == 136 || rate == 144 || rate == 168;
    if (n <= wave_max || !standard) {
        launch("k_sponge_raw", k_sponge_raw_w, n, WAVE, st, n, msg, rate, nblocks, out, outlen, out_stride);
        return 0;
    }
    if (out_stride & 3) return -1;
    const size_t grid = ceil_div(n, WAVE);
    switch (rate) {
    case 72: launch("k_sponge_raw", k_sponge_raw<72>, grid, WAVE, st, n, msg, nblocks, out, outlen, out_stride); break;
    case 104: launch("k_sponge_raw", k_sponge_raw<104>, grid, WAVE, st, n, msg, nblocks, out, outlen, out_stride); break;
    case 136: launch("k_sponge_raw", k_sponge_raw<136>, grid, WAVE, st, n, msg, nblocks, out, outlen, out_stride); break;
    case 144: launch("k_sponge_raw", k_sponge_raw<144>, grid, WAVE, st, n, msg, nblocks, out, outlen, out_stride); break;
    case 168: launch("k_sponge_raw", k_sponge_raw<168>, grid, WAVE, st, n, msg, nblocks, out, outlen, out_stride); break;
    default: return -1;
    }
    return 0;
}

}
```

### crystals-kyber_amd/csrc/mlkem_selftest.hpp

```cpp
#pragma once
#include "mlkem_arith.hpp"
#include "mlkem_rntt.hpp"
#include "mlkem_kpke2.hpp"

namespace mlkem {

__device__ __forceinline__ int imod_q(long long v) {
    int r = (int)(v % KQ);
    return r < 0 ? r + KQ : r;
}
__device__ __forceinline__ bool centred_ok(float t, long long exact) {
    const int ti = (int)t;
    return (float)ti == t && ti <= 1665 && ti >= -1665 && imod_q(exact - ti) == 0;
}

template <int D>
__device__ __forceinline__ unsigned compress_ref(int x) {
    const unsigned c = (unsigned)imod_q(x);
    const unsigned num = c << D, quo = num / (unsigned)KQ, rem = num % (unsigned)KQ;
    return (quo + (rem > (unsigned)(KQ / 2) ? 1u : 0u)) & ((1u << D) - 1u);
}
template <int D>
__device__ __forceinline__ unsigned compress_bad(int x) { return compress_f<D>((float)x) != compress_ref<D>(x) ? 1u : 0u; }

__global__ void __launch_bounds__(256) k_selftest(int sweep, unsigned long long* __restrict__ bad_out) {
    const size_t tid = (size_t)blockIdx.x * blockDim.x + threadIdx.x, nthreads = (size_t)gridDim.x * blockDim.x;
    unsigned long long bad = 0;
    if (sweep == 0) {
        for (long long i = (long long)tid; i <= (1ll << 25); i += (long long)nthreads) {
            const long long x = i - (1ll << 24);
            if (!centred_ok(fred((float)x), x)) bad++;
        }
    } else if (sweep == 1) {
        const long long per = 2 * 10082 + 1, total = 260 * per;
        for (long long i = (long long)tid; i < total; i += (long long)nthreads) {
            const int wi = (int)(i / per), b = (int)(i % per) - 10082;
            Tw w = (wi >> 1) < 128 ? ZETA_F.z[wi >> 1] : (wi >> 1) == 128 ? F_INV128 : F_INV128_Z1;
            if (wi & 1) w = tw_neg(w);
            const long long exact = (long long)(int)w.z * b;
            if (!centred_ok(fmulmod_shoup(w, (float)b), exact)) bad++;
            if (!centred_ok(fmulmod(w.z, (float)b), exact)) bad++;
            if (!centred_ok(fmulmod(w, (float)b), exact)) bad++;
        }
    } else if (sweep == 2) {
        for (long long i = (long long)tid; i < 8191; i += (long long)nthreads) {
            const int x = (int)i - 4095;
            bad += compress_bad<1>(x) + compress_bad<2>(x) + compress_bad<3>(x) + compress_bad<4>(x) + compress_bad<5>(x) +
                   compress_bad<6>(x) + compress_bad<7>(x) + compress_bad<8>(x) + compress_bad<9>(x) + compress_bad<10>(x) +
                   compress_bad<11>(x);
        }
    } else if (sweep == 3) {
        for (uint32_t t = (uint32_t)tid; t < 65536u; t += (uint32_t)nthreads) {
            float x[4];
            cbd_eval_f<2>(t, x);
#pragma unroll
            for (int m = 0; m < 4; m++) {
                const uint32_t n = (t >> (4 * m)) & 15u;
                const int want = (int)((n & 1) + ((n >> 1) & 1)) - (int)(((n >> 2) & 1) + ((n >> 3) & 1));
                if (x[m] != (float)want) bad++;
            }
        }
    } else if (sweep == 4) {
        for (size_t t = tid; t < ((size_t)1 << 24); t += nthreads) {
            float x[4];
            cbd_eval_f<3>((uint32_t)t, x);
#pragma unroll
            for (int m = 0; m < 4; m++) {
                const uint32_t n = ((uint32_t)t >> (6 * m)) & 63u;
                const int want = (int)__builtin_popcount(n & 7u) - (int)__builtin_popcount(n >> 3);
                if (x[m] != (float)want) bad++;
            }
        }
    } else if (sweep == 5) {
        const long long ny = 2 * 1665 + 1, total = 4096 * ny * 8;
        for (long long i = (long long)tid; i < total; i += (long long)nthreads) {
            const int corner = (int)(i & 7);
            const long long j = i >> 3;
            const int a0 = (int)(j / ny), y = (int)(j % ny) - 1665;
            const int a1 = (corner & 1) ? 4095 : 0, g = (corner & 2) ? 1665 : -1665, acc = (corner & 4) ? 1665 : -1665;
            const long long exact = (long long)a1 * g + (long long)a0 * y + acc;
            if (!centred_ok(basemul_term((float)acc, (float)a0, (float)y, (float)a1, (float)g), exact)) bad++;
            if (!centred_ok(basemul_term((float)acc, (float)a1, (float)g, (float)a0, (float)y), exact)) bad++;
        }
    } else if (sweep == 6) {
        for (long long i = (long long)tid; i <= (1ll << 21); i += (long long)nthreads) {
            const long long x = i - (1ll << 20);
            const int want = imod_q(x);
            if (fcanon((float)x) != want) bad++;
            const float c = fcanon_floor((float)x);
            if (c != (float)want) bad++;
        }
    }
    else if (sweep == 7) {
        for (long long i = (long long)tid; i <= (1ll << 23); i += (long long)nthreads) {
            const long long x = i - (1ll << 22);
            if (!centred_ok(fmulmod_shoup(TW_ONE, (float)x), x)) bad++;
        }
    }
    else if (sweep == 8) {
        for (long long i = (long long)tid; i <= (1ll << 24); i += (long long)nthreads) {
            const v2f r = fred2(v2f{(float)i, (float)-i});
            if (!centred_ok(r.x, i) || !centred_ok(r.y, -i)) bad++;
        }
        const long long per = 2 * 10082 + 1, total = 260 * per;
        for (long long i = (long long)tid; i < total; i += (long long)nthreads) {
            const int wi = (int)(i / per), b = (int)(i % per) - 10082;
            Tw w = (wi >> 1) < 128 ? ZETA_F.z[wi >> 1] : (wi >> 1) == 128 ? F_INV128 : F_INV128_Z1;
            if (wi & 1) w = tw_neg(w);
            const v2f r = fmulmod_shoup2(w, v2f{(float)b, (float)-b});
            if (!centred_ok(r.x, (long long)(int)w.z * b) || !centred_ok(r.y, -(long long)(int)w.z * b)) bad++;
        }
        for (long long i = (long long)tid; i <= 8190; i += (long long)nthreads) {
            const int x = (int)i - 4095;
            const v2f in[4] = {v2f{(float)x, (float)-x}, v2f{(float)x, (float)x}, v2f{(float)-x, (float)x}, v2f{0.f, (float)x}};
            unsigned c[8];
            k2_compress4<4>(in, c);
            if (c[0] != compress_ref<4>(x) || c[1] != compress_ref<4>(-x) || c[2] != c[0] || c[3] != c[0] || c[4] != c[1] || c[7] != c[0]) bad++;
            k2_compress4<5>(in, c);
            if (c[0] != compress_ref<5>(x) || c[1] != compress_ref<5>(-x) || c[5] != c[0]) bad++;
            k2_compress4<10>(in, c);
            if (c[0] != compress_ref<10>(x) || c[1] != compress_ref<10>(-x) || c[3] != c[0]) bad++;
            k2_compress4<11>(in, c);
            if (c[0] != compress_ref<11>(x) || c[1] != compress_ref<11>(-x) || c[4] != c[1]) bad++;
            const v2f inb[4] = {v2f{(float)(x + 2), (float)(2 - x)}, v2f{(float)(x + 2), (float)(x + 2)}, v2f{(float)(2 - x), (float)(x + 2)}, v2f{2.f, (float)(x + 2)}};
            k2_compress4<4, true>(inb, c);
            if (c[0] != compress_ref<4>(x) || c[1] != compress_ref<4>(-x) || c[2] != c[0] || c[4] != c[1] || c[6] != 0u || c[7] != c[0]) bad++;
            k2_compress4<5, true>(inb, c);
            if (c[0] != compress_ref<5>(x) || c[1] != compress_ref<5>(-x) || c[5] != c[0]) bad++;
            k2_compress4<10, true>(inb, c);
            if (c[0] != compress_ref<10>(x) || c[1] != compress_ref<10>(-x) || c[3] != c[0]) bad++;
            k2_compress4<11, true>(inb, c);
            if (c[0] != compress_ref<11>(x) || c[1] != compress_ref<11>(-x) || c[4] != c[1]) bad++;
        }
        for (long long i = (long long)tid; i <= (1ll << 20); i += (long long)nthreads) {
            const v2f in[4] = {v2f{(float)i, (float)-i}, v2f{(float)-i, (float)i}, v2f{(float)i, (float)i}, v2f{0.f, (float)-i}};
            unsigned c[8];
            k2_canon(in, c);
            const unsigned p = (unsigned)imod_q(i), m = (unsigned)imod_q(-i);
            if (c[0] != p || c[1] != m || c[2] != m || c[3] != p || c[4] != p || c[5] != p || c[6] != 0u || c[7] != m) bad++;
        }
        for (long long i = (long long)tid; i < (1ll << 16) * 6; i += (long long)nthreads) {
            const uint32_t v = (uint32_t)(i & 0xFFFF), fill = (uint32_t)((i >> 16) % 3) * 0x5A5Au + ((i >> 16) % 3 == 2 ? 0xFFFFu - 2 * 0x5A5Au : 0u);
            const bool upper = (i >> 16) >= 3;
            const uint32_t t = upper ? (v << 16) | fill : v | (fill << 16);
            v2f p[4], pb[4];
            k2_cbd2_eval8<false>(t, p);
            k2_cbd2_eval8<true>(t, pb);
            for (int j = 0; j < 4; j++)
                if (pb[j].x != p[j].x + 2.0f || pb[j].y != p[j].y + 2.0f) bad++;
            const float got[8] = {p[0].x, p[0].y, p[1].x, p[1].y, p[2].x, p[2].y, p[3].x, p[3].y};
            for (int c = 0; c < 8; c++) {
                const uint32_t nib = (t >> (4 * c)) & 0xFu;
                const int want = (int)((nib & 1u) + ((nib >> 1) & 1u)) - (int)(((nib >> 2) & 1u) + ((nib >> 3) & 1u));
                if (got[c] != (float)want) bad++;
            }
        }
        const long long na = 4096, ny = 2 * 1665 + 1;
        for (long long i = (long long)tid; i < na * ny * 8; i += (long long)nthreads) {
            const int corner = (int)(i / (na * ny));
            const long long r = i % (na * ny);
            const int a0 = (int)(r / ny), y0 = (int)(r % ny) - 1665;
            const int a1 = (corner & 1) ? 4095 : 0, g = (corner & 2) ? 1665 : -1665, ac = (corner & 4) ? 1665 : -1665;
            v2f acc[4], a[4], y[4];
            float yg[4];
            for (int j = 0; j < 4; j++) { acc[j] = v2f{(float)ac, (float)ac}; a[j] = v2f{(float)a0, (float)a1}; y[j] = v2f{(float)y0, (float)g}; yg[j] = (float)g; }
            k2_basemul_acc(acc, a, y, yg);
            const long long e0 = (long long)a0 * y0 + (long long)a1 * g + ac, e1 = (long long)a0 * g + (long long)a1 * y0 + ac;
            if (!centred_ok(acc[0].x, e0) || !centred_ok(acc[0].y, e1) || !centred_ok(acc[3].x, e0) || !centred_ok(acc[3].y, e1)) bad++;
        }
    }
    for (int off = 32; off > 0; off >>= 1) bad += __shfl_xor(bad, off);
    if ((threadIdx.x & 63) == 0 && bad) atomicAdd(bad_out, bad);
}

constexpr int SELFTEST_SWEEPS = 9;

}
```

### crystals-kyber_amd/csrc/mlkem_small.hpp

```cpp
#pragma once
#include "mlkem_wkeccak.hpp"
#include "mlkem_kpke2.hpp"
#include "mlkem_kpke4.hpp"

namespace mlkem {

constexpr int SMALL_WAVES = 8, SMALL_WAVES_DENSE = 4, SMALL_WAVES_WIDE = 12;

__device__ __forceinline__ unsigned take_job(uint32_t* counter) {
    unsigned j = 0;
    if (lane_id_fresh() == 0) j = atomicAdd(counter, 1u);
#ifdef MLKEM_EMU
    return (unsigned)__shfl((int)j, 0);
#else
    return (unsigned)__builtin_amdgcn_readfirstlane((int)j);
#endif
}

#ifdef MLKEM_EMU
__device__ __forceinline__ void block_barrier() { emu::block_barrier(); }
__device__ __forceinline__ void wave_global_fence() { emu::wave_barrier(); }
#else
__device__ __forceinline__ void block_barrier() { __syncthreads(); }
__device__ __forceinline__ void wave_global_fence() { __threadfence_block(); }
#endif

constexpr int XOF_LDS_WORDS = 44;

template <int QB = KQ, int CAP = SAMPLE_CAP>
__device__ __forceinline__ unsigned wk_sample_ntt_seed(const WkLane& c, uint2 seed, unsigned i0, unsigned i1, uint16_t* poly, uint32_t* sq) {
    static_assert(CAP > 224 && CAP <= 280, "the limit falls into the fifth squeeze block");
    const int i = wk_index();
    const bool prim = wk_primary();
    const unsigned l = (unsigned)lane_id();
    if (!(i >= 0 && i < 4)) { seed.x = 0; seed.y = 0; }
    const unsigned bo = 3u * l, w = bo >> 2, sh = 8u * (bo & 3u);
    const unsigned long long below = (1ull << l) - 1ull;
    unsigned retries = 0;
    for (;;) {
        WkState a;
        a.lo = seed.x; a.hi = seed.y;
        if (i == 4) a.lo = (i0 & 0xFFu) | ((i1 & 0xFFu) << 8) | (0x1Fu << 16);
        if (i == 20) a.hi = 0x80000000u;
        unsigned cnt = 0;
#pragma unroll 1
        for (int blk = 0; blk < 5 && cnt < 256u; blk++) {
            wk_permute(a, c);
            if (prim && i < 21) { sq[2 * i] = a.lo; sq[2 * i + 1] = a.hi; }
            wave_lds_fence();
            uint32_t v = 0;
            if (l < 56u) v = __builtin_amdgcn_alignbit(sq[w + 1], sq[w], sh) & 0xFFFFFFu;
            wave_lds_fence();
            const unsigned ntr = blk == 4 ? (unsigned)(CAP - 224) : 56u;
            const unsigned d1 = v & 0xFFFu, d2 = v >> 12;
            const bool ok1 = l < ntr && d1 < (unsigned)QB, ok2 = l < ntr && d2 < (unsigned)QB;
            const unsigned long long m1 = __ballot(ok1), m2 = __ballot(ok2);
            const unsigned pos1 = cnt + (unsigned)__builtin_popcountll(m1 & below) + (unsigned)__builtin_popcountll(m2 & below);
            const unsigned pos2 = pos1 + (ok1 ? 1u : 0u);
            if (ok1 && pos1 < 256u) poly[pos1] = (uint16_t)d1;
            if (ok2 && pos2 < 256u) poly[pos2] = (uint16_t)d2;
            cnt += (unsigned)__builtin_popcountll(m1) + (unsigned)__builtin_popcountll(m2);
        }
        if (cnt >= 256u) break;
        i0 = (i0 + 1u) & 0xFFu;
        i1 = (i1 + 1u) & 0xFFu;
        retries++;
    }
    return retries;
}

template <int QB = KQ, int CAP = SAMPLE_CAP>
__device__ __forceinline__ void wk_sample_ntt(const WkLane& c, const uint8_t* rho, unsigned i0, unsigned i1, uint16_t* poly, uint32_t* sq) {
    const int i = wk_index();
    uint2 seed;
    seed.x = 0; seed.y = 0;
    if (i >= 0 && i < 4) seed = reinterpret_cast<const uint2*>(rho)[i];
    wk_sample_ntt_seed<QB, CAP>(c, seed, i0, i1, poly, sq);
}
template <int QB = KQ, int CAP = SAMPLE_CAP>
__global__ void __launch_bounds__(WAVE) k_sample_ntt_w(size_t n, const uint8_t* __restrict__ seeds34, uint16_t* __restrict__ out, uint8_t* __restrict__ retries) {
    __shared__ uint32_t sq[XOF_LDS_WORDS];
    __shared__ uint2 rc_table[WK_RC_ENTRIES];
    const size_t g = blockIdx.x;
    if (g >= n) return;
    const uint8_t* sp = seeds34 + g * 34;
    const int i = wk_index();
    uint2 seed;
    seed.x = 0; seed.y = 0;
    if (i >= 0 && i < 4) {
        const uint8_t* b = sp + 8 * i;
        seed.x = (uint32_t)b[0] | ((uint32_t)b[1] << 8) | ((uint32_t)b[2] << 16) | ((uint32_t)b[3] << 24);
        seed.y = (uint32_t)b[4] | ((uint32_t)b[5] << 8) | ((uint32_t)b[6] << 16) | ((uint32_t)b[7] << 24);
    }
    WkLane c;
    wk_lane_init(c, rc_table);
    const unsigned r = wk_sample_ntt_seed<QB, CAP>(c, seed, sp[32], sp[33], out + g * 256, sq);
    if (retries && lane_id() == 0) retries[g] = (uint8_t)(r < 255u ? r : 255u);
}

__global__ void __launch_bounds__(WAVE) k_sponge_raw_w(size_t n, const uint8_t* __restrict__ msg, unsigned rate, unsigned nblocks,
                                                       uint8_t* __restrict__ out, unsigned outlen, size_t out_stride) {
    __shared__ uint2 rc_table[WK_RC_ENTRIES];
    const size_t g = blockIdx.x;
    if (g >= n) return;
    WkLane c;
    wk_lane_init(c, rc_table);
    const int i = wk_index();
    const unsigned base = 8u * (unsigned)(i < 0 ? 0 : i);
    const uint8_t* m = msg + g * (size_t)nblocks * rate;
    WkState a;
    a.lo = 0; a.hi = 0;
    for (unsigned blk = 0; blk < nblocks; blk++) {
        if (i >= 0) {
#pragma unroll
            for (unsigned b = 0; b < 8; b++)
                if (base + b < rate) {
                    const uint32_t v = m[(size_t)blk * rate + base + b];
                    if (b < 4) a.lo ^= v << (8 * b);
                    else a.hi ^= v << (8 * (b - 4));
                }
        }
        wk_permute(a, c);
    }
    uint8_t* o = out + g * out_stride;
    for (unsigned done = 0; done < outlen; done += rate) {
        if (done) wk_permute(a, c);
        const unsigned take = outlen - done < rate ? outlen - done : rate;
        if (wk_primary()) {
#pragma unroll
            for (unsigned b = 0; b < 8; b++)
                if (base + b < take) o[done + base + b] = (uint8_t)((b < 4 ? a.lo >> (8 * b) : a.hi >> (8 * (b - 4))) & 0xFFu);
        }
    }
}

__device__ __forceinline__ void wk_prf(const WkLane& c, const uint8_t* r32, unsigned ctr, unsigned eta, unsigned rate, uint8_t* out) {
    const int i = wk_index();
    const bool prim = wk_primary();
    WkState a;
    a.lo = 0; a.hi = 0;
    if (i >= 0 && i < 4) {
        const uint2 v = reinterpret_cast<const uint2*>(r32)[i];
        a.lo = v.x; a.hi = v.y;
    }
    if (i == 4) a.lo = (ctr & 0xFFu) | (0x1Fu << 8);
    const int nq = (int)(rate / 8u), want = (int)(8u * eta);
    if (i == nq - 1) a.hi ^= 0x80000000u;
    wk_permute(a, c);
    uint2 o;
    o.x = a.lo; o.y = a.hi;
    if (prim && i < (want < nq ? want : nq)) reinterpret_cast<uint2*>(out)[i] = o;
    if (want > nq) {
        wk_permute(a, c);
        o.x = a.lo; o.y = a.hi;
        if (prim && i < want - nq) reinterpret_cast<uint2*>(out)[nq + i] = o;
    }
}

template <int K, int ETA1>
struct __attribute__((aligned(16))) SmallHand {
    uint16_t A[K * K * 256];
    uint8_t prf[(2 * K + 1) * (ETA1 == 3 ? 192 : 128)];
    uint8_t r[32], m[32], Kp[32], Kbar[32], rho[32];
};

struct SmallSync {
    uint32_t next_job;
    uint32_t jobs_done;
    uint32_t r_ready;
    uint32_t kbar_ready;
};

template <int K, int ETA1, int ETA_REST = 2>
__device__ __forceinline__ void small_jobs(SmallSync& sy, const WkLane& cst, const uint8_t* rho, bool transpose, uint16_t* A, const uint8_t* key,
                                           uint8_t* prf, int rows, unsigned prf_rate, uint32_t* sq) {
    constexpr unsigned PS = (ETA1 == 3) ? 192 : 128;
    for (unsigned j; (j = take_job(&sy.next_job)) < (unsigned)(K * K + rows);) {
        if (j < (unsigned)(K * K)) {
            wk_sample_ntt(cst, rho, transpose ? j / K : j % K, transpose ? j % K : j / K, A + j * 256, sq);
        } else {
            const unsigned row = j - K * K;
            flag_wait(&sy.r_ready, 1u);
            wk_prf(cst, key, row, row < (unsigned)K ? (unsigned)ETA1 : (unsigned)ETA_REST, prf_rate, prf + row * PS);
        }
        flag_signal(&sy.jobs_done);
    }
}

__device__ __forceinline__ void wk_H(WkState& a, const WkLane& c, const uint8_t* msg, unsigned len) {
    wk_absorb<136, 0x06>(a, c, msg, len, msg, len);
}

template <int K, int ETA1, int DU, int DV, int NW>
__global__ void __launch_bounds__(WAVE * NW)
k_encaps_small(size_t n, const uint8_t* __restrict__ ek, const uint8_t* __restrict__ m, uint8_t* __restrict__ c, uint8_t* __restrict__ Kout,
               int32_t* __restrict__ mod_status, int prf_rate) {
    __shared__ K2Lds<K + 1> xl;
    __shared__ SmallHand<K, ETA1> hand;
    __shared__ uint32_t sq[NW][XOF_LDS_WORDS];
    __shared__ uint2 rc_tables[NW][WK_RC_ENTRIES];
    __shared__ SmallSync sy;
    constexpr unsigned EK = 384 * K + 32, CLEN = 32 * (DU * K + DV);
    const int wv = wave_id();
    const size_t item = blockIdx.x;
    if (item >= n) return;
    const uint8_t* my_ek = ek + item * EK;
    uint16_t* my_A = hand.A;
    uint8_t *my_prf = hand.prf, *my_r = hand.r;
    WkLane cst;
    wk_lane_init(cst, rc_tables[wave_id()]);
    if (threadIdx.x == 0) { sy.next_job = 0; sy.jobs_done = 0; sy.r_ready = 0; sy.kbar_ready = 0; }
    block_barrier();
    if (wv == 0) {
        const int i = wk_index();
        WkState a;
        wk_H(a, cst, my_ek, EK);
        uint2 mv;
        mv.x = 0; mv.y = 0;
        if (i >= 0 && i < 4) mv = reinterpret_cast<const uint2*>(m + item * 32)[i];
        wk_G_of_x_and_digest(a, cst, mv);
        uint2 o;
        o.x = a.lo; o.y = a.hi;
        if (wk_primary() && i < 4) reinterpret_cast<uint2*>(Kout + item * 32)[i] = o;
        else if (wk_primary() && i < 8) reinterpret_cast<uint2*>(my_r)[i - 4] = o;
        flag_signal(&sy.r_ready);
    }
    small_jobs<K, ETA1>(sy, cst, my_ek + 384 * K, true, my_A, my_r, my_prf, 2 * K + 1, (unsigned)prf_rate, sq[wv]);
    if (wv != 0) return;
    flag_wait(&sy.jobs_done, (uint32_t)(K * K + 2 * K + 1));
    encrypt1_body<K, ETA1, DU, DV, false>(xl.xch, my_ek, m + item * 32, my_A, my_prf, c + item * CLEN, nullptr, nullptr, nullptr, nullptr,
                                          mod_status ? mod_status + item : nullptr);
}

template <int K, int ETA1, int DU, int DV, bool HASH_CHECK, int JRATE, int NW>
__global__ void __launch_bounds__(WAVE * NW)
k_decaps_small(size_t n, const uint8_t* __restrict__ dk, const uint8_t* __restrict__ c, uint8_t* __restrict__ Kout, int32_t* __restrict__ status,
               int prf_rate) {
    __shared__ K2Lds<K + 1> xl;
    __shared__ SmallHand<K, ETA1> hand;
    __shared__ uint32_t sq[NW][XOF_LDS_WORDS];
    __shared__ uint2 rc_tables[NW][WK_RC_ENTRIES];
    __shared__ SmallSync sy;
    constexpr unsigned EK = 384 * K + 32, DK = 768 * K + 96, CLEN = 32 * (DU * K + DV);
    const int wv = wave_id();
    const bool check_block = HASH_CHECK && blockIdx.x < n;
    const size_t item = HASH_CHECK && !check_block ? blockIdx.x - n : blockIdx.x;
    if (item >= n || (check_block && wv != 0)) return;
    const uint8_t* my_dk = dk + item * DK;
    const uint8_t* my_c = c + item * CLEN;
    uint16_t* my_A = hand.A;
    uint8_t *my_prf = hand.prf, *my_r = hand.r, *my_m = hand.m, *my_Kp = hand.Kp, *my_Kbar = hand.Kbar;
    WkLane cst;
    wk_lane_init(cst, rc_tables[wave_id()]);
    const int i = wk_index();
    const bool prim = wk_primary();
    if (check_block) {
        WkState a;
        wk_H(a, cst, my_dk + 384 * K, EK);
        uint2 h;
        h.x = 0; h.y = 0;
        if (prim && i < 4) h = reinterpret_cast<const uint2*>(my_dk + 768 * K + 32)[i];
        const bool differ = prim && i < 4 && (h.x != a.lo || h.y != a.hi);
        const bool bad = __ballot(differ) != 0;
        if (lane_id() == 0 && status) status[item] = bad ? -5 : 0;
        return;
    }
    if (threadIdx.x == 0) { sy.next_job = 0; sy.jobs_done = 0; sy.r_ready = 0; sy.kbar_ready = 0; }
    block_barrier();
    if (wv == 0) {
        decrypt4_body<K, DU, DV>(0, 1, my_dk, (size_t)DK, my_c, my_m);
        wave_global_fence();
        uint2 v;
        v.x = 0; v.y = 0;
        if (i >= 0 && i < 4) v = reinterpret_cast<const uint2*>(my_m)[i];
        else if (i >= 4 && i < 8) v = reinterpret_cast<const uint2*>(my_dk + 768 * K + 32)[i - 4];
        WkState a;
        a.lo = v.x; a.hi = v.y;
        if (i == 8) { a.lo = 0x06u; a.hi = 0x80000000u; }
        wk_permute(a, cst);
        uint2 o;
        o.x = a.lo; o.y = a.hi;
        if (prim && i < 4) reinterpret_cast<uint2*>(my_Kp)[i] = o;
        else if (prim && i < 8) reinterpret_cast<uint2*>(my_r)[i - 4] = o;
        if (!HASH_CHECK && lane_id() == 0 && status) status[item] = 0;
        flag_signal(&sy.r_ready);
    } else if (wv == 1) {
        WkState a;
        wk_absorb<JRATE, 0x1F>(a, cst, my_dk + 768 * K + 64, 32, my_c, 32 + CLEN);
        uint2 o;
        o.x = a.lo; o.y = a.hi;
        if (prim && i < 4) reinterpret_cast<uint2*>(my_Kbar)[i] = o;
        flag_signal(&sy.kbar_ready);
    }
    small_jobs<K, ETA1>(sy, cst, my_dk + 768 * K, true, my_A, my_r, my_prf, 2 * K + 1, (unsigned)prf_rate, sq[wv]);
    if (wv != 0) return;
    flag_wait(&sy.jobs_done, (uint32_t)(K * K + 2 * K + 1));
    encrypt1_body<K, ETA1, DU, DV, true>(xl.xch, my_dk + 384 * K, my_m, my_A, my_prf, nullptr, my_c, my_Kp, my_Kbar, Kout + item * 32, nullptr,
                                         &sy.kbar_ready);
}

template <int K, int ETA1, bool KEM_DK, int NW>
__global__ void __launch_bounds__(WAVE * NW)
k_keygen_small(size_t n, const uint8_t* __restrict__ d, const uint8_t* __restrict__ z, uint8_t* ek, uint8_t* dk, int prf_rate) {
    __shared__ K2Lds<K> xl;
    __shared__ SmallHand<K, ETA1> hand;
    __shared__ uint32_t sq[NW][XOF_LDS_WORDS];
    __shared__ uint2 rc_tables[NW][WK_RC_ENTRIES];
    __shared__ SmallSync sy;
    constexpr unsigned EK = 384 * K + 32, DK = KEM_DK ? 768 * K + 96 : 384 * K;
    const int wv = wave_id();
    const size_t item = blockIdx.x;
    if (item >= n) return;
    uint8_t *my_ek = ek + item * EK, *my_dk = dk + item * DK;
    uint16_t* my_A = hand.A;
    uint8_t *my_prf = hand.prf, *my_rho = hand.rho, *my_sigma = hand.r;
    WkLane cst;
    wk_lane_init(cst, rc_tables[wave_id()]);
    const int i = wk_index();
    const bool prim = wk_primary();
    if (wv == 0) {
        WkState a;
        a.lo = 0; a.hi = 0;
        if (i >= 0 && i < 4) {
            const uint2 v = reinterpret_cast<const uint2*>(d + item * 32)[i];
            a.lo = v.x; a.hi = v.y;
        }
        if (i == 4) a.lo = (unsigned)K | (0x06u << 8);
        if (i == 8) a.hi = 0x80000000u;
        wk_permute(a, cst);
        uint2 o;
        o.x = a.lo; o.y = a.hi;
        if (prim && i < 4) reinterpret_cast<uint2*>(my_rho)[i] = o;
        else if (prim && i < 8) reinterpret_cast<uint2*>(my_sigma)[i - 4] = o;
    }
    if (threadIdx.x == 0) { sy.next_job = 0; sy.jobs_done = 0; sy.r_ready = 1; sy.kbar_ready = 0; }
    block_barrier();
    small_jobs<K, ETA1, ETA1>(sy, cst, my_rho, false, my_A, my_sigma, my_prf, 2 * K, (unsigned)prf_rate, sq[wv]);
    block_barrier();
    if (wv == 0) {
        keygen2_body<K, ETA1, KEM_DK>(xl.xch, 0, 1, my_A, my_prf, my_rho, my_ek, my_dk);
        if constexpr (KEM_DK) {
            wave_global_fence();
            WkState a;
            wk_H(a, cst, my_ek, EK);
            uint2 o;
            o.x = a.lo; o.y = a.hi;
            if (i >= 4 && i < 8) o = reinterpret_cast<const uint2*>(z + item * 32)[i - 4];
            if (prim && i < 8) reinterpret_cast<uint2*>(my_dk + 768 * K + 32)[i] = o;
        }
    }
}

template <int K>
struct __attribute__((aligned(16))) SeedLds {
    uint8_t ek[384 * K + 32];
    uint8_t s[384 * K];
    uint8_t h[32];
};
struct SeedSync {
    SmallSync kg;
    SmallSync enc;
    uint32_t ek_ready, h_ready;
};

template <class T>
__device__ __forceinline__ void wave_zero_lds(T& obj) {
    static_assert(sizeof(T) % 16 == 0, "whole 16-byte stores");
    uint4 z;
    z.x = 0; z.y = 0; z.z = 0; z.w = 0;
    uint4* p = reinterpret_cast<uint4*>(&obj);
    constexpr unsigned N = (unsigned)(sizeof(T) / 16);
#pragma unroll 1
    for (unsigned o0 = 0; o0 < N; o0 += WAVE) {
        const unsigned o = o0 + (unsigned)lane_id();
        if (o < N) p[o] = z;
    }
}

template <int K, int ETA1, int DU, int DV, int JRATE, int NW>
__global__ void __launch_bounds__(WAVE * NW)
k_decaps_seed_small(size_t n, const uint8_t* __restrict__ seed, const uint8_t* __restrict__ c, uint8_t* __restrict__ Kout, int prf_rate) {
    static_assert(NW >= 4, "roles of waves 0, 1 and 2");
    __shared__ K2Lds<K + 1> xl;
    __shared__ SmallHand<K, ETA1> hand;
    __shared__ SeedLds<K> kl;
    __shared__ uint32_t sq[NW][XOF_LDS_WORDS];
    __shared__ uint2 rc_tables[NW][WK_RC_ENTRIES];
    __shared__ SeedSync sy;
    constexpr unsigned EK = 384 * K + 32, CLEN = 32 * (DU * K + DV);
    const int wv = wave_id();
    const size_t item = blockIdx.x;
    if (item >= n) return;
    const uint8_t* my_seed = seed + item * 64;
    const uint8_t* my_c = c + item * CLEN;
    WkLane cst;
    wk_lane_init(cst, rc_tables[wave_id()]);
    const int i = wk_index();
    const bool prim = wk_primary();
    if (wv == 0) {
        WkState a;
        a.lo = 0; a.hi = 0;
        if (i >= 0 && i < 4) {
            const uint2 v = reinterpret_cast<const uint2*>(my_seed)[i];
            a.lo = v.x; a.hi = v.y;
        }
        if (i == 4) a.lo = (unsigned)K | (0x06u << 8);
        if (i == 8) a.hi = 0x80000000u;
        wk_permute(a, cst);
        uint2 o;
        o.x = a.lo; o.y = a.hi;
        if (prim && i < 4) reinterpret_cast<uint2*>(hand.rho)[i] = o;
        else if (prim && i < 8) reinterpret_cast<uint2*>(hand.r)[i - 4] = o;
    }
    if (threadIdx.x == 0) {
        sy.kg.next_job = 0; sy.kg.jobs_done = 0; sy.kg.r_ready = 1; sy.kg.kbar_ready = 0;
        sy.enc.next_job = 0; sy.enc.jobs_done = 0; sy.enc.r_ready = 0; sy.enc.kbar_ready = 0;
        sy.ek_ready = 0; sy.h_ready = 0;
    }
    block_barrier();
    small_jobs<K, ETA1, ETA1>(sy.kg, cst, hand.rho, false, hand.A, hand.r, hand.prf, 2 * K, (unsigned)prf_rate, sq[wv]);
    block_barrier();
    if (wv == 0) {
        keygen2_body<K, ETA1, false>(xl.xch, 0, 1, hand.A, hand.prf, hand.rho, kl.ek, kl.s);
        wave_global_fence();
        flag_signal(&sy.ek_ready);
        decrypt4_body<K, DU, DV>(0, 1, kl.s, (size_t)(384 * K), my_c, hand.m);
        wave_global_fence();
        flag_wait(&sy.h_ready, 1u);
        uint2 v;
        v.x = 0; v.y = 0;
        if (i >= 0 && i < 4) v = reinterpret_cast<const uint2*>(hand.m)[i];
        else if (i >= 4 && i < 8) v = reinterpret_cast<const uint2*>(kl.h)[i - 4];
        WkState a;
        a.lo = v.x; a.hi = v.y;
        if (i == 8) { a.lo = 0x06u; a.hi = 0x80000000u; }
        wk_permute(a, cst);
        uint2 o;
        o.x = a.lo; o.y = a.hi;
        if (prim && i < 4) reinterpret_cast<uint2*>(hand.Kp)[i] = o;
        else if (prim && i < 8) reinterpret_cast<uint2*>(hand.r)[i - 4] = o;
        flag_signal(&sy.enc.r_ready);
    } else if (wv == 1) {
        WkState a;
        wk_absorb<JRATE, 0x1F>(a, cst, my_seed + 32, 32, my_c, 32 + CLEN);
        uint2 o;
        o.x = a.lo; o.y = a.hi;
        if (prim && i < 4) reinterpret_cast<uint2*>(hand.Kbar)[i] = o;
        flag_signal(&sy.enc.kbar_ready);
    } else if (wv == 2) {
        flag_wait(&sy.ek_ready, 1u);
        WkState a;
        wk_H(a, cst, kl.ek, EK);
        uint2 o;
        o.x = a.lo; o.y = a.hi;
        if (prim && i < 4) reinterpret_cast<uint2*>(kl.h)[i] = o;
        flag_signal(&sy.h_ready);
    }
    if (wv != 0) {
        constexpr unsigned PS = (ETA1 == 3) ? 192 : 128;
#pragma unroll 1
        for (unsigned row = (unsigned)wv - 1; row < (unsigned)(2 * K + 1); row += NW - 1) {
            flag_wait(&sy.enc.r_ready, 1u);
            wk_prf(cst, hand.r, row, row < (unsigned)K ? (unsigned)ETA1 : 2u, (unsigned)prf_rate, hand.prf + row * PS);
            flag_signal(&sy.enc.jobs_done);
        }
        return;
    }
    flag_wait(&sy.enc.jobs_done, (uint32_t)(2 * K + 1));
    encrypt1_body<K, ETA1, DU, DV, true, true>(xl.xch, kl.ek, hand.m, hand.A, hand.prf, nullptr, my_c, hand.Kp, hand.Kbar,
                                                       Kout + item * 32, nullptr, &sy.enc.kbar_ready);
    wave_lds_fence();
    wave_zero_lds(hand);
    wave_zero_lds(kl);
    wave_zero_lds(xl);
    wave_zero_lds(sq);
#ifdef MLKEM_EMU_LDS_PROBE
    if (lane_id() == 0) {
        MLKEM_EMU_LDS_PROBE(&hand, sizeof hand); MLKEM_EMU_LDS_PROBE(&kl, sizeof kl);
        MLKEM_EMU_LDS_PROBE(&xl, sizeof xl); MLKEM_EMU_LDS_PROBE(&sq, sizeof sq);
    }
#endif
}

}
```

Before: 61.01 million.

## Defer modular reductions in basemul rows and specialize status checks at compile time

Replaces the per-product modular reduction in the NTT-domain basemul accumulation with a row routine that reduces only every two or three products, relying on fp32 exact-integer headroom. The final inverse-NTT layer now uses the regular hi layer, and the 1/128 scaling moves into a Shoup multiply on the forward-NTT outputs. A STATUS template parameter removes the modulus-range check and ballot when no status buffer is requested. Exactness now depends on tighter magnitude bounds, which new self-test sweeps exercise.

Measured after the change: 61.32 million, median of 6. No clear change (+0.5%).

```diff
diff --git a/crystals-kyber_amd/csrc/mlkem_keyset.hpp b/crystals-kyber_amd/csrc/mlkem_keyset.hpp
--- a/crystals-kyber_amd/csrc/mlkem_keyset.hpp
+++ b/crystals-kyber_amd/csrc/mlkem_keyset.hpp
@@ -109,7 +109,7 @@
     if (item0 >= n) return;
     const size_t h = (size_t)(lane_id() >> 5), item = item0 + h < n ? item0 + h : item0;
     const size_t key = keyset_key(idx, n_keys, item);
-    encrypt2_body<K, ETA1, DU, DV, COMPARE>(lds_all[wv].xch, item0, n, ek + key * ek_stride, 0, msg, At + key * (size_t)(K * K * 256), prf,
+    encrypt2_body<K, ETA1, DU, DV, COMPARE, false>(lds_all[wv].xch, item0, n, ek + key * ek_stride, 0, msg, At + key * (size_t)(K * K * 256), prf,
                                             c_out, c_in, Kp, Kbar, Kout, (int32_t*)nullptr, 0);
 }
 
@@ -200,7 +200,7 @@
     small_jobs<K, ETA1>(sy, cst, nullptr, true, nullptr, hand.r, hand.prf, 2 * K + 1, (unsigned)prf_rate, nullptr);
     if (wv != 0) return;
     flag_wait(&sy.jobs_done, (uint32_t)(2 * K + 1));
-    encrypt1_body<K, ETA1, DU, DV, false>(xl.xch, my_ek, m + item * 32, At + key * (size_t)(K * K * 256), hand.prf, c + item * CLEN, nullptr,
+    encrypt1_body<K, ETA1, DU, DV, false, false>(xl.xch, my_ek, m + item * 32, At + key * (size_t)(K * K * 256), hand.prf, c + item * CLEN, nullptr,
                                           nullptr, nullptr, nullptr, nullptr);
     if (lane_id() == 0 && status) status[item] = 0;
     wave_lds_fence();
@@ -265,7 +265,7 @@
     small_jobs<K, ETA1>(sy, cst, nullptr, true, nullptr, hand.r, hand.prf, 2 * K + 1, (unsigned)prf_rate, nullptr);
     if (wv != 0) return;
     flag_wait(&sy.jobs_done, (uint32_t)(2 * K + 1));
-    encrypt1_body<K, ETA1, DU, DV, true>(xl.xch, my_dk + 384 * K, hand.m, At + key * (size_t)(K * K * 256), hand.prf, nullptr, my_c, hand.Kp,
+    encrypt1_body<K, ETA1, DU, DV, true, false>(xl.xch, my_dk + 384 * K, hand.m, At + key * (size_t)(K * K * 256), hand.prf, nullptr, my_c, hand.Kp,
                                          hand.Kbar, Kout + item * 32, nullptr, &sy.kbar_ready);
     if (lane_id() == 0 && status) status[item] = 0;
     wave_lds_fence();
diff --git a/crystals-kyber_amd/csrc/mlkem_kpke2.hpp b/crystals-kyber_amd/csrc/mlkem_kpke2.hpp
--- a/crystals-kyber_amd/csrc/mlkem_kpke2.hpp
+++ b/crystals-kyber_amd/csrc/mlkem_kpke2.hpp
@@ -170,24 +170,7 @@
     k2_fred_pairs<NP, 0, 1>(p);
     k2_exchange<K2_LB, K2_LA, NP>(xch, h, t, p);
     k2_layer_lo<NP, true>(p, FZ3, FZ2);
-    {
-        v2f sm[2 * NP], df[2 * NP];
-        Tw zs[2 * NP], zd[2 * NP];
-#pragma unroll
-        for (int q = 0; q < NP; q++)
-#pragma unroll
-            for (int m = 0; m < 2; m++) {
-                sm[2 * q + m] = p[q][m] + p[q][m + 2];
-                df[2 * q + m] = p[q][m + 2] - p[q][m];
-                zs[2 * q + m] = F_INV128; zd[2 * q + m] = F_INV128_Z1;
-            }
-        k2_shoup_n<2 * NP>(zs, sm);
-        k2_shoup_n<2 * NP>(zd, df);
-#pragma unroll
-        for (int q = 0; q < NP; q++)
-#pragma unroll
-            for (int m = 0; m < 2; m++) { p[q][m] = sm[2 * q + m]; p[q][m + 2] = df[2 * q + m]; }
-    }
+    k2_layer_hi<NP, true>(p, FZ1);
     k2_exchange<K2_LA, K2_NAT, NP>(xch, h, t, p);
 }
 
@@ -245,18 +228,27 @@
     yg[2] = fmulmod_shoup(d1, y[2].y);
     yg[3] = fmulmod_shoup(tw_neg(d1), y[3].y);
 }
-__device__ __forceinline__ void k2_basemul_acc(v2f (&acc)[4], const v2f (&a)[4], const v2f (&y)[4], const float (&yg)[4]) {
-    v2f c[4];
-#pragma unroll
-    for (int j = 0; j < 4; j++) c[j] = fma2(splat2(a[j].x), y[j], acc[j]);
-#pragma unroll
-    for (int j = 0; j < 4; j++) {
-        c[j].x = __builtin_fmaf(a[j].y, yg[j], c[j].x);
-        c[j].y = __builtin_fmaf(a[j].y, y[j].x, c[j].y);
-    }
-    k2_fred_n<4>(c);
-#pragma unroll
-    for (int j = 0; j < 4; j++) acc[j] = c[j];
+template <int K, int PER, bool FINAL, class GetA>
+__device__ __forceinline__ void k2_basemul_row(v2f (&acc)[4], GetA&& get_a, const v2f (&y)[K][4], const float (&yg)[K][4]) {
+    static_assert(PER == 2 || PER == 3, "products between two reductions");
+#pragma unroll
+    for (int b = 0; b < K; b++) {
+        v2f av[4];
+        get_a(b, av);
+        if (b > 0 && (2 * b) % PER == 0) k2_fred_n<4>(acc);
+#pragma unroll
+        for (int j = 0; j < 4; j++) {
+            if (b == 0) acc[j] = fma2(splat2(av[j].x), y[b][j], splat2(0.f));
+            else acc[j] = fma2(splat2(av[j].x), y[b][j], acc[j]);
+        }
+        if ((2 * b + 1) % PER == 0) k2_fred_n<4>(acc);
+#pragma unroll
+        for (int j = 0; j < 4; j++) {
+            acc[j].x = __builtin_fmaf(av[j].y, yg[b][j], acc[j].x);
+            acc[j].y = __builtin_fmaf(av[j].y, y[b][j].x, acc[j].y);
+        }
+    }
+    if constexpr (FINAL) k2_fred_n<4>(acc);
 }
 
 __device__ __forceinline__ void k2_unpack16(const uint4 v, v2f (&p)[4]) {
@@ -406,7 +398,7 @@
     return 0;
 }
 
-template <int K, int ETA1, int DU, int DV, bool COMPARE>
+template <int K, int ETA1, int DU, int DV, bool COMPARE, bool STATUS>
 __device__ __forceinline__ void
 encrypt2_body(float2 (*xch)[2][128], size_t item0, size_t n, const uint8_t* __restrict__ ek, size_t ek_stride, const uint8_t* __restrict__ msg,
               const uint16_t* __restrict__ A, const uint8_t* __restrict__ prf, uint8_t* __restrict__ c_out, const uint8_t* __restrict__ c_in,
@@ -449,9 +441,10 @@
 #pragma unroll
         for (int b = 0; b < K; b++) k2_cbd_eval<ETA1>(raw_y[b], yh[b]);
         k2_ntt<K>(yh, xch, h, t, tw);
+        const Tw inv128[4] = {F_INV128, F_INV128, F_INV128, F_INV128};
 #pragma unroll
         for (int b = 0; b < K; b++) {
-            k2_fred_n<4>(yh[b]);
+            k2_shoup_n<4>(inv128, yh[b]);
             k2_gamma(yh[b], tw.d0, tw.d1, yg[b]);
         }
     }
@@ -463,19 +456,16 @@
     K2Piece<DV> cv_ref;
 #pragma unroll
     for (int a = 0; a < NG; a++) {
-#pragma unroll
-        for (int j = 0; j < 4; j++) acc[a][j] = splat2(0.f);
-#pragma unroll
-        for (int b = 0; b < K; b++) {
-            v2f av[4];
-            if (a < K) {
-                k2_unpack16(a_all[a][b], av);
-            } else {
+        if (a < K) {
+            k2_basemul_row<K, 3, true>(acc[a], [&](int b, v2f (&av)[4]) { k2_unpack16(a_all[a][b], av); }, yh, yg);
+        } else {
+            k2_basemul_row<K, 2, true>(acc[a], [&](int b, v2f (&av)[4]) {
                 k2_decode12(a_all[a][b].x, a_all[a][b].y, a_all[a][b].z, av);
-#pragma unroll
-                for (int j = 0; j < 4; j++) over = over || (av[j].x >= F_Q) || (av[j].y >= F_Q);
-            }
-            k2_basemul_acc(acc[a], av, yh[b], yg[b]);
+                if constexpr (STATUS) {
+#pragma unroll
+                    for (int j = 0; j < 4; j++) over = over || (av[j].x >= F_Q) || (av[j].y >= F_Q);
+                }
+            }, yh, yg);
         }
     }
     if constexpr (COMPARE) {
@@ -505,7 +495,7 @@
             diff |= k2_emit<DV, COMPARE, true>(acc[a], nb, COMPARE ? nullptr : my_c + K * 32 * DU, cv_ref, valid);
         }
     }
-    if (mod_status) {
+    if constexpr (STATUS) {
         const unsigned long long bal = __ballot(over);
         const bool bad = ((bal >> (32 * h)) & 0xFFFFFFFFull) != 0;
         if (t == 0 && valid) mod_status[item] = bad ? -4 : 0;
@@ -520,7 +510,7 @@
         }
     }
 }
-template <int K, int ETA1, int DU, int DV, bool COMPARE, bool A_T = false>
+template <int K, int ETA1, int DU, int DV, bool COMPARE, bool STATUS, bool A_T = false>
 __device__ __forceinline__ void
 encrypt1_body(float2 (*xch)[2][128], const uint8_t* __restrict__ ek, const uint8_t* __restrict__ msg, const uint16_t* __restrict__ A,
               const uint8_t* __restrict__ prf, uint8_t* __restrict__ c_out, const uint8_t* __restrict__ c_in, const uint8_t* __restrict__ Kp,
@@ -561,9 +551,10 @@
 #pragma unroll
         for (int b = 0; b < K; b++) k2_cbd_eval<ETA1>(raw_y[b], yh[b]);
         k2_ntt<K>(yh, xch, h, t, tw);
+        const Tw inv128[4] = {F_INV128, F_INV128, F_INV128, F_INV128};
 #pragma unroll
         for (int b = 0; b < K; b++) {
-            k2_fred_n<4>(yh[b]);
+            k2_shoup_n<4>(inv128, yh[b]);
             k2_gamma(yh[b], tw.d0, tw.d1, yg[b]);
         }
     }
@@ -575,20 +566,19 @@
 #pragma unroll
     for (int i = 0; i < NL; i++) {
         const bool is_v = kind(i) == 2 || (kind(i) == 1 && h == 1);
-#pragma unroll
-        for (int j = 0; j < 4; j++) acc[i][j] = splat2(0.f);
-#pragma unroll
-        for (int b = 0; b < K; b++) {
-            v2f av[4];
+        auto get_a = [&](int b, v2f (&av)[4]) {
             if (is_v) {
                 k2_decode12(a_all[i][b].x, a_all[i][b].y, a_all[i][b].z, av);
-#pragma unroll
-                for (int j = 0; j < 4; j++) over = over || (av[j].x >= F_Q) || (av[j].y >= F_Q);
+                if constexpr (STATUS) {
+#pragma unroll
+                    for (int j = 0; j < 4; j++) over = over || (av[j].x >= F_Q) || (av[j].y >= F_Q);
+                }
             } else {
                 k2_unpack16(a_all[i][b], av);
             }
-            k2_basemul_acc(acc[i], av, yh[b], yg[b]);
-        }
+        };
+        if (kind(i) == 0) k2_basemul_row<K, 3, true>(acc[i], get_a, yh, yg);
+        else k2_basemul_row<K, 2, true>(acc[i], get_a, yh, yg);
     }
     if constexpr (COMPARE) {
 #pragma unroll
@@ -622,7 +612,7 @@
             diff |= k2_emit<DU, COMPARE, true>(acc[i], nb, COMPARE ? nullptr : c_out + a * 32 * DU, cu_ref[i], store);
         }
     }
-    if (mod_status) {
+    if constexpr (STATUS) {
         const bool bad = __ballot(over) != 0;
         if (l == 0) mod_status[0] = bad ? -4 : 0;
     }
@@ -637,7 +627,7 @@
     }
 }
 
-template <int K, int ETA1, int DU, int DV, bool COMPARE>
+template <int K, int ETA1, int DU, int DV, bool STATUS, bool COMPARE>
 __global__ void __launch_bounds__(WAVE * KPKE2_WAVES, kpke2_minwaves(K))
 k_encrypt2(size_t n, const uint8_t* __restrict__ ek, size_t ek_stride, const uint8_t* __restrict__ msg, const uint16_t* __restrict__ A,
            const uint8_t* __restrict__ prf, uint8_t* __restrict__ c_out, const uint8_t* __restrict__ c_in, const uint8_t* __restrict__ Kp,
@@ -646,7 +636,7 @@
     const int wv = wave_id();
     const size_t item0 = 2 * ((size_t)blockIdx.x * KPKE2_WAVES + wv);
     if (item0 >= n) return;
-    encrypt2_body<K, ETA1, DU, DV, COMPARE>(lds_all[wv].xch, item0, n, ek, ek_stride, msg, A, prf, c_out, c_in, Kp, Kbar, Kout, mod_status, a_stride);
+    encrypt2_body<K, ETA1, DU, DV, COMPARE, STATUS>(lds_all[wv].xch, item0, n, ek, ek_stride, msg, A, prf, c_out, c_in, Kp, Kbar, Kout, mod_status, a_stride);
 }
 
 __device__ __forceinline__ void k2_canon(const v2f (&p)[4], unsigned (&c)[8]) {
@@ -711,14 +701,11 @@
     k2_ntt<K>(eh, xch, h, t, tw);
 #pragma unroll
     for (int a = 0; a < K; a++) {
-        v2f acc[4] = {splat2(0.f), splat2(0.f), splat2(0.f), splat2(0.f)};
-#pragma unroll
-        for (int b = 0; b < K; b++) {
-            v2f av[4];
+        v2f acc[4];
+        k2_basemul_row<K, 3, false>(acc, [&](int b, v2f (&av)[4]) {
             if constexpr (!PF) a_all[a][b] = *reinterpret_cast<const uint4*>(my_A + (a * K + b) * 256 + 8 * nb);
             k2_unpack16(a_all[a][b], av);
-            k2_basemul_acc(acc, av, sh[b], sg[b]);
-        }
+        }, sh, sg);
 #pragma unroll
         for (int j = 0; j < 4; j++) acc[j] = acc[j] + eh[a][j];
         unsigned c[8];
diff --git a/crystals-kyber_amd/csrc/mlkem_pipeline.hpp b/crystals-kyber_amd/csrc/mlkem_pipeline.hpp
--- a/crystals-kyber_amd/csrc/mlkem_pipeline.hpp
+++ b/crystals-kyber_amd/csrc/mlkem_pipeline.hpp
@@ -174,9 +174,18 @@
     launch_sample_split<QB, CAP>(st, p, n, n, rho, rho_stride, transpose, r, prf_per_item, n_eta1, ws);
 }
 
+template <class T, class... Rest>
+inline bool encrypt_wants_status(T first, Rest... rest) {
+    if constexpr (sizeof...(Rest) == 1) return first != nullptr;
+    else return encrypt_wants_status(rest...);
+}
 template <int K, int ETA1, int DU, int DV, bool CMP, class... Args>
 inline void encrypt_launch(const char* label, stream_t st, size_t n, Args... args) {
-    launch(label, k_encrypt2<K, ETA1, DU, DV, CMP>, ceil_div(ceil_div(n, 2), KPKE2_WAVES), WAVE * KPKE2_WAVES, st, n, args...);
+    const size_t grid = ceil_div(ceil_div(n, 2), KPKE2_WAVES);
+    bool status = false;
+    if constexpr (!CMP) status = encrypt_wants_status(args...);
+    if (!status) launch(label, k_encrypt2<K, ETA1, DU, DV, false, CMP>, grid, WAVE * KPKE2_WAVES, st, n, args...);
+    else if constexpr (!CMP) launch(label, k_encrypt2<K, ETA1, DU, DV, true, false>, grid, WAVE * KPKE2_WAVES, st, n, args...);
 }
 
 template <int K, int ETA1>
@@ -223,10 +232,13 @@
     if (n == 0) return;
     if (!r_user && n <= ws.small_max(K)) {
         const int rate = ws.fips ? 136 : 168;
-        if (n <= ws.small_lat_max)
-            launch("k_encaps_small", k_encaps_small<K, ETA1, DU, DV, SMALL_WAVES>, n, WAVE * SMALL_WAVES, st, n, ek, m, c, Kout, mod_status, rate);
-        else
-            launch("k_encaps_small", k_encaps_small<K, ETA1, DU, DV, SMALL_WAVES_DENSE>, n, WAVE * SMALL_WAVES_DENSE, st, n, ek, m, c, Kout, mod_status, rate);
+#define MLKEM_ES(NW, ST) launch("k_encaps_small", k_encaps_small<K, ETA1, DU, DV, NW, ST>, n, WAVE * NW, st, n, ek, m, c, Kout, mod_status, rate)
+        const bool lat = n <= ws.small_lat_max;
+        if (lat && mod_status) MLKEM_ES(SMALL_WAVES, true);
+        else if (lat) MLKEM_ES(SMALL_WAVES, false);
+        else if (mod_status) MLKEM_ES(SMALL_WAVES_DENSE, true);
+        else MLKEM_ES(SMALL_WAVES_DENSE, false);
+#undef MLKEM_ES
         return;
     }
     SideFork fork(ws, st, r_user ? (size_t)-1 : n);
diff --git a/crystals-kyber_amd/csrc/mlkem_selftest.hpp b/crystals-kyber_amd/csrc/mlkem_selftest.hpp
--- a/crystals-kyber_amd/csrc/mlkem_selftest.hpp
+++ b/crystals-kyber_amd/csrc/mlkem_selftest.hpp
@@ -22,6 +22,47 @@
 }
 template <int D>
 __device__ __forceinline__ unsigned compress_bad(int x) { return compress_f<D>((float)x) != compress_ref<D>(x) ? 1u : 0u; }
+
+template <int K, int PER, bool FINAL>
+__device__ __forceinline__ unsigned basemul_row_bad(int a0, int a1, int y0, int g, bool alt) {
+    v2f a[K][4], y[K][4], acc[4];
+    float yg[K][4];
+    long long e0 = 0, e1 = 0;
+    for (int b = 0; b < K; b++) {
+        const int sg = (alt && (b & 1)) ? -1 : 1;
+        for (int j = 0; j < 4; j++) { a[b][j] = v2f{(float)a0, (float)a1}; y[b][j] = v2f{(float)(sg * y0), (float)(sg * g)}; yg[b][j] = (float)(sg * g); }
+        e0 += (long long)sg * ((long long)a0 * y0 + (long long)a1 * g);
+        e1 += (long long)sg * ((long long)a0 * g + (long long)a1 * y0);
+    }
+    k2_basemul_row<K, PER, FINAL>(acc, [&](int b, v2f (&av)[4]) { for (int j = 0; j < 4; j++) av[j] = a[b][j]; }, y, yg);
+    if constexpr (FINAL) {
+        return (!centred_ok(acc[0].x, e0) || !centred_ok(acc[0].y, e1) || !centred_ok(acc[3].x, e0) || !centred_ok(acc[3].y, e1)) ? 1u : 0u;
+    } else {
+        const int eh = g > 0 ? 11679 : -11679;
+        for (int j = 0; j < 4; j++) acc[j] = acc[j] + splat2((float)eh);
+        unsigned c[8];
+        k2_canon(acc, c);
+        return (c[0] != (unsigned)imod_q(e0 + eh) || c[1] != (unsigned)imod_q(e1 + eh) || c[6] != c[0] || c[7] != c[1]) ? 1u : 0u;
+    }
+}
+template <int K>
+__device__ __forceinline__ unsigned long long basemul_row_sweep(size_t tid, size_t nthreads) {
+    unsigned long long bad = 0;
+    const long long ny = 2 * 1668 + 1;
+    for (long long i = (long long)tid; i < 4096 * ny * 8; i += (long long)nthreads) {
+        const int corner = (int)(i / (4096 * ny));
+        const long long r = i % (4096 * ny);
+        const int a0 = (int)(r / ny), y0 = (int)(r % ny) - 1668;
+        const int g = (corner & 2) ? 1668 : -1668;
+        const bool alt = (corner & 4) != 0;
+        bad += basemul_row_bad<K, 2, true>(a0, (corner & 1) ? 4095 : 0, y0, g, alt);
+        if (a0 <= 3328) {
+            bad += basemul_row_bad<K, 3, true>(a0, (corner & 1) ? 3328 : 0, y0, g, alt);
+            bad += basemul_row_bad<K, 3, false>(a0, (corner & 1) ? 3328 : 0, y0, g, alt);
+        }
+    }
+    return bad;
+}
 
 __global__ void __launch_bounds__(256) k_selftest(int sweep, unsigned long long* __restrict__ bad_out) {
     const size_t tid = (size_t)blockIdx.x * blockDim.x + threadIdx.x, nthreads = (size_t)gridDim.x * blockDim.x;
@@ -110,8 +151,9 @@
             const v2f r = fmulmod_shoup2(w, v2f{(float)b, (float)-b});
             if (!centred_ok(r.x, (long long)(int)w.z * b) || !centred_ok(r.y, -(long long)(int)w.z * b)) bad++;
         }
-        for (long long i = (long long)tid; i <= 8190; i += (long long)nthreads) {
-            const int x = (int)i - 4095;
+        for (long long i = (long long)tid; i <= 2 * 16383; i += (long long)nthreads) {
+            const int x = (int)i - 16383;
+            const bool du = x >= -8191 && x <= 8191;
             const v2f in[4] = {v2f{(float)x, (float)-x}, v2f{(float)x, (float)x}, v2f{(float)-x, (float)x}, v2f{0.f, (float)x}};
             unsigned c[8];
             k2_compress4<4>(in, c);
@@ -119,18 +161,18 @@
             k2_compress4<5>(in, c);
             if (c[0] != compress_ref<5>(x) || c[1] != compress_ref<5>(-x) || c[5] != c[0]) bad++;
             k2_compress4<10>(in, c);
-            if (c[0] != compress_ref<10>(x) || c[1] != compress_ref<10>(-x) || c[3] != c[0]) bad++;
+            if (du && (c[0] != compress_ref<10>(x) || c[1] != compress_ref<10>(-x) || c[3] != c[0])) bad++;
             k2_compress4<11>(in, c);
-            if (c[0] != compress_ref<11>(x) || c[1] != compress_ref<11>(-x) || c[4] != c[1]) bad++;
+            if (du && (c[0] != compress_ref<11>(x) || c[1] != compress_ref<11>(-x) || c[4] != c[1])) bad++;
             const v2f inb[4] = {v2f{(float)(x + 2), (float)(2 - x)}, v2f{(float)(x + 2), (float)(x + 2)}, v2f{(float)(2 - x), (float)(x + 2)}, v2f{2.f, (float)(x + 2)}};
             k2_compress4<4, true>(inb, c);
             if (c[0] != compress_ref<4>(x) || c[1] != compress_ref<4>(-x) || c[2] != c[0] || c[4] != c[1] || c[6] != 0u || c[7] != c[0]) bad++;
             k2_compress4<5, true>(inb, c);
             if (c[0] != compress_ref<5>(x) || c[1] != compress_ref<5>(-x) || c[5] != c[0]) bad++;
             k2_compress4<10, true>(inb, c);
-            if (c[0] != compress_ref<10>(x) || c[1] != compress_ref<10>(-x) || c[3] != c[0]) bad++;
+            if (du && (c[0] != compress_ref<10>(x) || c[1] != compress_ref<10>(-x) || c[3] != c[0])) bad++;
             k2_compress4<11, true>(inb, c);
-            if (c[0] != compress_ref<11>(x) || c[1] != compress_ref<11>(-x) || c[4] != c[1]) bad++;
+            if (du && (c[0] != compress_ref<11>(x) || c[1] != compress_ref<11>(-x) || c[4] != c[1])) bad++;
         }
         for (long long i = (long long)tid; i <= (1ll << 20); i += (long long)nthreads) {
             const v2f in[4] = {v2f{(float)i, (float)-i}, v2f{(float)-i, (float)i}, v2f{(float)i, (float)i}, v2f{0.f, (float)-i}};
@@ -155,19 +197,16 @@
                 if (got[c] != (float)want) bad++;
             }
         }
-        const long long na = 4096, ny = 2 * 1665 + 1;
-        for (long long i = (long long)tid; i < na * ny * 8; i += (long long)nthreads) {
-            const int corner = (int)(i / (na * ny));
-            const long long r = i % (na * ny);
-            const int a0 = (int)(r / ny), y0 = (int)(r % ny) - 1665;
-            const int a1 = (corner & 1) ? 4095 : 0, g = (corner & 2) ? 1665 : -1665, ac = (corner & 4) ? 1665 : -1665;
-            v2f acc[4], a[4], y[4];
-            float yg[4];
-            for (int j = 0; j < 4; j++) { acc[j] = v2f{(float)ac, (float)ac}; a[j] = v2f{(float)a0, (float)a1}; y[j] = v2f{(float)y0, (float)g}; yg[j] = (float)g; }
-            k2_basemul_acc(acc, a, y, yg);
-            const long long e0 = (long long)a0 * y0 + (long long)a1 * g + ac, e1 = (long long)a0 * g + (long long)a1 * y0 + ac;
-            if (!centred_ok(acc[0].x, e0) || !centred_ok(acc[0].y, e1) || !centred_ok(acc[3].x, e0) || !centred_ok(acc[3].y, e1)) bad++;
-        }
+        for (long long i = (long long)tid; i <= (1ll << 15); i += (long long)nthreads) {
+            const int b = (int)i - (1 << 14);
+            const Tw zz[1] = {F_INV128};
+            v2f r[1] = {v2f{(float)b, (float)-b}};
+            k2_shoup_n<1>(zz, r);
+            const int rx = (int)r[0].x, ry = (int)r[0].y;
+            if ((float)rx != r[0].x || (float)ry != r[0].y || rx > 1668 || rx < -1668 || ry > 1668 || ry < -1668 ||
+                imod_q((long long)(int)F_INV128.z * b - rx) != 0 || imod_q(-(long long)(int)F_INV128.z * b - ry) != 0) bad++;
+        }
+        bad += basemul_row_sweep<2>(tid, nthreads) + basemul_row_sweep<3>(tid, nthreads) + basemul_row_sweep<4>(tid, nthreads);
     }
     for (int off = 32; off > 0; off >>= 1) bad += __shfl_xor(bad, off);
     if ((threadIdx.x & 63) == 0 && bad) atomicAdd(bad_out, bad);
diff --git a/crystals-kyber_amd/csrc/mlkem_small.hpp b/crystals-kyber_amd/csrc/mlkem_small.hpp
--- a/crystals-kyber_amd/csrc/mlkem_small.hpp
+++ b/crystals-kyber_amd/csrc/mlkem_small.hpp
@@ -191,7 +191,7 @@
     wk_absorb<136, 0x06>(a, c, msg, len, msg, len);
 }
 
-template <int K, int ETA1, int DU, int DV, int NW>
+template <int K, int ETA1, int DU, int DV, int NW, bool STATUS>
 __global__ void __launch_bounds__(WAVE * NW)
 k_encaps_small(size_t n, const uint8_t* __restrict__ ek, const uint8_t* __restrict__ m, uint8_t* __restrict__ c, uint8_t* __restrict__ Kout,
                int32_t* __restrict__ mod_status, int prf_rate) {
@@ -228,8 +228,8 @@
     small_jobs<K, ETA1>(sy, cst, my_ek + 384 * K, true, my_A, my_r, my_prf, 2 * K + 1, (unsigned)prf_rate, sq[wv]);
     if (wv != 0) return;
     flag_wait(&sy.jobs_done, (uint32_t)(K * K + 2 * K + 1));
-    encrypt1_body<K, ETA1, DU, DV, false>(xl.xch, my_ek, m + item * 32, my_A, my_prf, c + item * CLEN, nullptr, nullptr, nullptr, nullptr,
-                                          mod_status ? mod_status + item : nullptr);
+    encrypt1_body<K, ETA1, DU, DV, false, STATUS>(xl.xch, my_ek, m + item * 32, my_A, my_prf, c + item * CLEN, nullptr, nullptr, nullptr, nullptr,
+                                                  STATUS ? mod_status + item : nullptr);
 }
 
 template <int K, int ETA1, int DU, int DV, bool HASH_CHECK, int JRATE, int NW>
@@ -295,7 +295,7 @@
     small_jobs<K, ETA1>(sy, cst, my_dk + 768 * K, true, my_A, my_r, my_prf, 2 * K + 1, (unsigned)prf_rate, sq[wv]);
     if (wv != 0) return;
     flag_wait(&sy.jobs_done, (uint32_t)(K * K + 2 * K + 1));
-    encrypt1_body<K, ETA1, DU, DV, true>(xl.xch, my_dk + 384 * K, my_m, my_A, my_prf, nullptr, my_c, my_Kp, my_Kbar, Kout + item * 32, nullptr,
+    encrypt1_body<K, ETA1, DU, DV, true, false>(xl.xch, my_dk + 384 * K, my_m, my_A, my_prf, nullptr, my_c, my_Kp, my_Kbar, Kout + item * 32, nullptr,
                                          &sy.kbar_ready);
 }
 
@@ -467,7 +467,7 @@
         return;
     }
     flag_wait(&sy.enc.jobs_done, (uint32_t)(2 * K + 1));
-    encrypt1_body<K, ETA1, DU, DV, true, true>(xl.xch, kl.ek, hand.m, hand.A, hand.prf, nullptr, my_c, hand.Kp, hand.Kbar,
+    encrypt1_body<K, ETA1, DU, DV, true, false, true>(xl.xch, kl.ek, hand.m, hand.A, hand.prf, nullptr, my_c, hand.Kp, hand.Kbar,
                                                        Kout + item * 32, nullptr, &sy.enc.kbar_ready);
     wave_lds_fence();
     wave_zero_lds(hand);
```
